# PlatonB/ld-tools

Measured on AMD Instinct MI355X. Metric: SNP-pairs/sec (r2+D'), higher is better.
Workload: dtype fp4 (E2M1 0/1 operands, exact f32 accumulation)

## Files before the change

### include/ldx.h

```cpp
#ifndef LDX_H
#define LDX_H

#include <stddef.h>
#include <stdint.h>

#ifdef __cplusplus
extern "C" {
#endif

#define LDX_VERSION 102
#define LDX_SLAB_ROWS 128u
#define LDX_GROUP_ROWS 8u
#define LDX_CHUNK_HAPS 128u
#define LDX_UNIT_PAIRS (LDX_SLAB_ROWS * LDX_GROUP_ROWS)
#define LDX_CELL_OFFSET4(r8, c) ((r8) * LDX_SLAB_ROWS + (((c) & 31u) << 2) + ((c) >> 5))
#define LDX_CELL_OFFSET8(r8, c) ((r8) * LDX_SLAB_ROWS + (((c) >> 6) << 6) + (((c) & 31u) << 1) + (((c) >> 5) & 1u))
#define LDX_CELL_OFFSET(out_format, r8, c) ((out_format) == LDX_OUT_LD32 ? LDX_CELL_OFFSET8(r8, c) : LDX_CELL_OFFSET4(r8, c))
#define LDX_MAX_HAPS 10240u

#define LDX_OK 0
#define LDX_E_ARG (-1)
#define LDX_E_HIP (-2)
#define LDX_E_UNSUPPORTED (-3)
#define LDX_E_OVERFLOW (-4)
// ... 4 lines not shown

#define LDX_MEASURE_RSQ 0
#define LDX_MEASURE_DPRIME 1

typedef struct { float r_square; float d_prime; } ldx_ld32;
typedef struct { uint16_t r_square; uint16_t d_prime; } ldx_k16;
typedef struct { double r_square; double d_prime; } ldx_ld64;
#define LDX_LD32_BIG_BITS 0x7FC00B16u
#define LDX_K16_INT0 0x8000u
#define LDX_K16_BIG 0x7FFFu
#define LDX_OUT_LD32 0
#define LDX_OUT_K16 1
typedef struct { uint16_t value; } ldx_k16one;
#define LDX_OUT_K16_RSQ 2
#define LDX_OUT_K16_DPRIME 3
typedef struct { float r; } ldx_r32;
#define LDX_OUT_R32 4

typedef struct {
    uint32_t query;
    uint32_t oppos;
    float r_square;
    float d_prime;
} ldx_hit;

int ldx_version(void);
const char *ldx_last_error(void);
int ldx_device_count(void);
int ldx_device_arch(int device, char *buf, size_t buflen);

uint32_t ldx_n_slabs(uint32_t n_snps);
uint32_t ldx_n_chunks(uint32_t n_hap);
size_t ldx_plane_bytes(uint32_t n_snps, uint32_t n_hap);
uint32_t ldx_padded_snps(uint32_t n_snps);
uint64_t ldx_triangle_units(uint32_t n_snps);
uint64_t ldx_triangle_unit_of(uint32_t n_snps, uint32_t row, uint32_t col);
uint64_t ldx_triangle_tile_base(uint32_t n_snps, uint32_t tile);
uint64_t ldx_triangle_cell_index(uint32_t n_snps, uint32_t row, uint32_t col, int out_format);

int ldx_pack_codes_dev(const int8_t *codes, uint32_t n_snps, uint32_t n_hap, size_t ld_codes,
                       void *alt, void *ref, uint32_t *acnt, uint32_t *rcnt, void *stream);
int ldx_tile_plane_dev(const uint32_t *rowmajor, uint32_t n_snps, uint32_t n_hap, size_t ld_words,
                       void *tiled, uint32_t *cnt, void *stream);
int ldx_snp_stats_dev(const uint32_t *acnt, const uint32_t *rcnt, uint32_t n_snps, uint32_t n_hap,
                      double *fa, double *fr, double *q, void *stream);

int ldx_alt_freq4_dev(const uint32_t *acnt, uint32_t n_snps, uint32_t n_hap, double *freq4, void *stream);

int ldx_panel_select_dev(const void *alt_src, const void *ref_src, uint32_t n_snps_src, uint32_t n_hap_src,
                         const uint32_t *snp_idx, uint32_t n_snps_dst, const uint32_t *hap_idx, uint32_t n_hap_dst,
                         void *alt_dst, void *ref_dst, uint32_t *acnt_dst, uint32_t *rcnt_dst, void *stream);

int ldx_bed_unpack_dev(const uint8_t *bed, size_t row_bytes, uint32_t n_ind_src, uint32_t n_rows,
                       const uint32_t *ind_idx, uint32_t n_ind_dst, int alt_is_a2, uint32_t row0, uint32_t n_snps_panel,
                       void *alt, void *ref, uint32_t *acnt, uint32_t *rcnt, void *stream);
int ldx_bed_pack_dev(const void *alt, const void *ref, uint32_t n_snps, uint32_t n_hap, uint32_t row0, uint32_t n_rows,
                     uint8_t *bed, size_t row_bytes, int alt_is_a2, void *stream);

int ldx_pair_counts_dev(const void *alt_i, uint32_t n_i, const void *alt_j, uint32_t n_j,
                        uint32_t n_hap, uint32_t *n11, size_t ld, void *stream);

int ldx_ld_from_counts_dev(uint32_t n, size_t m, const uint32_t *n11, const uint32_t *a1,
                           const uint32_t *r1, const uint32_t *a2, const uint32_t *r2,
                           ldx_ld64 *raw, ldx_ld32 *rounded, uint8_t *flags, void *stream);
int ldx_ld_from_counts_ex_dev(uint32_t n, size_t m, const uint32_t *n11, const uint32_t *a1,
                              const uint32_t *r1, const uint32_t *a2, const uint32_t *r2,
                              ldx_ld64 *raw, double *k, ldx_ld32 *cells32, ldx_k16 *cells16, uint8_t *flags,
                              void *stream);

int ldx_ld_pairs_dev(const void *alt, const uint32_t *acnt, const uint32_t *rcnt, uint32_t n_snps, uint32_t n_hap,
                     const uint32_t *rows, const uint32_t *cols, size_t m, double *k, ldx_ld64 *raw,
                     uint8_t *flags, uint32_t *n11, void *stream);

int ldx_triangle_dev(const void *alt, const double *fa, const double *fr, const double *q,
                     uint32_t n_snps, uint32_t n_hap, uint64_t unit_begin, uint64_t unit_end,
                     ldx_ld32 *out, ldx_ld64 *out_raw, uint32_t *out_n11, void *stream);
#define LDX_PATH_AUTO 0
#define LDX_PATH_POPCOUNT 1
#define LDX_PATH_MFMA 2
#define LDX_PATH_FP4 3
int ldx_set_triangle_path(int path);
int ldx_get_triangle_path(void);
size_t ldx_triangle_workspace_bytes(void);
int ldx_triangle_workspace_init_dev(void *workspace, size_t workspace_bytes, void *stream);
int ldx_triangle_ex_dev(const void *alt, const double *fa, const double *fr, const double *q,
                        uint32_t n_snps, uint32_t n_hap, uint64_t unit_begin, uint64_t unit_end,
                        int path, int out_format, void *out, ldx_ld64 *out_raw, uint32_t *out_n11,
                        void *workspace, size_t workspace_bytes, void *stream);

int ldx_triangle_dense_dev(const ldx_ld32 *strips, uint32_t n_snps, int measure, int has_thres,
                           double thres, uint32_t row_begin, uint32_t row_end, float *dense,
                           size_t ld, void *stream);
int ldx_triangle_dense_ex_dev(const void *strips, int strips_format, uint32_t n_snps, int measure, int has_thres,
                              double thres, uint32_t row_begin, uint32_t row_end, float *dense,
                              size_t ld, void *stream);
int ldx_triangle_r_block_dev(const ldx_r32 *strips, uint32_t n_snps, const uint32_t *acnt, const uint32_t *rcnt,
                             uint32_t n_hap, uint32_t row_begin, uint32_t row_end, uint32_t col_begin, uint32_t col_end,
                             float *out, size_t ld_out, void *stream);

int ldx_area_dev(const void *alt, const double *fa, const double *fr, const double *q,
                 uint32_t n_snps, uint32_t n_hap, const int64_t *positions,
                 const uint32_t *queries, uint32_t n_query, int64_t flank, int measure,
                 double thres, ldx_hit *hits, uint64_t hit_cap, uint64_t *n_hits, void *workspace,
                 size_t workspace_bytes, void *stream);
size_t ldx_area_workspace_bytes(uint32_t n_snps, uint32_t n_hap, uint32_t n_query);
int ldx_area_scan_dev(const void *alt, const double *fa, const double *fr, const double *q,
                      uint32_t n_snps, uint32_t n_hap, const int64_t *positions,
                      const uint32_t *queries, uint32_t n_query, int64_t flank, int measure,
                      double thres, ldx_hit *hits, uint64_t hit_cap, uint64_t *n_hits, uint32_t *query_counts,
                      void *workspace, size_t workspace_bytes, void *stream);
int ldx_area_finish_dev(ldx_hit *raw, const uint64_t *n_reserved, uint64_t hit_cap, uint32_t n_snps,
                        ldx_hit *sorted, uint32_t *offsets, uint64_t *summary, void *workspace,
                        size_t workspace_bytes, void *stream);
size_t ldx_area_finish_workspace_bytes(uint32_t n_snps);
int ldx_area_finish_ex_dev(ldx_hit *raw, const uint64_t *n_reserved, uint64_t hit_cap, uint32_t n_snps,
                           ldx_hit *sorted, uint32_t *offsets, uint64_t *summary, void *workspace,
                           size_t workspace_bytes, int counts_ready, void *stream);
uint32_t *ldx_area_finish_counts(void *finish_workspace);
int ldx_area_results_dev(const ldx_hit *sorted, uint64_t n_hits, int64_t *query, int64_t *oppos, float *values,
                         const uint32_t *offsets_src, uint32_t *offsets_dst, uint32_t n_offsets,
                         const uint32_t *word_src, uint32_t *word_dst, void *stream);
size_t ldx_area_band_passes_offset(uint32_t n_snps);
int ldx_set_area_path(int path);
int ldx_get_area_path(void);

size_t ldx_ld_score_workspace_bytes(uint32_t n_snps, uint32_t n_hap);
int ldx_ld_score_dev(const void *alt, const uint32_t *acnt, const uint32_t *rcnt, const double *fa, const double *fr,
                     uint32_t n_snps, uint32_t n_hap, const int64_t *positions, int64_t window,
                     const uint8_t *annot, uint32_t n_annot, int path,
                     uint64_t *sums, void *workspace, size_t workspace_bytes, void *stream);

#define LDX_DECAY_MAX_BINS 1024u
size_t ldx_ld_decay_workspace_bytes(uint32_t n_snps, uint32_t n_hap);
int ldx_ld_decay_dev(const void *alt, const uint32_t *acnt, const uint32_t *rcnt, const double *fa, const double *fr,
                     uint32_t n_snps, uint32_t n_hap, const int64_t *positions, int64_t window, int64_t bin_width,
                     const uint8_t *keep, int path,
                     uint64_t *sums, uint64_t *counts, uint32_t n_bins,
                     void *workspace, size_t workspace_bytes, void *stream);

size_t ldx_ld_fgt_workspace_bytes(uint32_t n_snps, uint32_t n_hap);
int ldx_ld_fgt_dev(const void *alt, const uint32_t *acnt, uint32_t n_snps, uint32_t n_hap, const int64_t *positions,
                   int64_t window, uint32_t min_count, const uint8_t *keep, int path,
                   uint32_t *left, void *workspace, size_t workspace_bytes, void *stream);
int ldx_ld_blocks_dev(const uint32_t *left, const int64_t *positions, const uint8_t *keep, uint32_t n_snps, int64_t window,
                      uint32_t *block_of, uint32_t *n_out, void *stream);

size_t ldx_ld_cross_workspace_bytes(uint32_t n_snps, uint32_t n_hap);
int ldx_ld_cross_dev(const void *alt, const uint32_t *acnt, const uint32_t *rcnt, const double *fa, const double *fr,
                     uint32_t n_snps, uint32_t n_hap, const int64_t *positions, int64_t window, int path,
                     uint64_t *sides, uint64_t *cross, void *workspace, size_t workspace_bytes, void *stream);
int ldx_ld_cross_scan_dev(const uint64_t *sides, uint32_t n_snps, uint64_t *cross, void *stream);
size_t ldx_ld_split_workspace_bytes(uint32_t n);
int ldx_ld_split_dev(const uint64_t *cross, uint32_t n, uint32_t min_snps, uint32_t max_snps,
                     uint32_t *cuts, uint32_t *n_out, void *workspace, size_t workspace_bytes, void *stream);

size_t ldx_ld_matvec_workspace_bytes(uint32_t n_snps, uint32_t n_hap);
int ldx_ld_matvec_dev(const void *alt, const uint32_t *acnt, const uint32_t *rcnt, const double *fa, const double *fr,
                      uint32_t n_snps, uint32_t n_hap, const int64_t *positions, int64_t window,
                      const float *x, uint32_t n_rhs, int power, int path,
                      int64_t *sums, void *workspace, size_t workspace_bytes, void *stream);

size_t ldx_ld_neighbors_workspace_bytes(uint32_t n_snps, uint32_t n_hap);
int ldx_ld_neighbors_dev(const void *alt, const uint32_t *acnt, const uint32_t *rcnt, const double *fa, const double *fr,
                         uint32_t n_snps, uint32_t n_hap, const int64_t *positions, int64_t window, float r2_bound, int path,
                         ldx_hit *hits, uint64_t hit_cap, uint64_t *n_hits, uint32_t *row_counts,
                         void *workspace, size_t workspace_bytes, void *stream);
// ... 94 lines not shown
                               const void *alt_j, const void *ref_j, const uint32_t *acnt_j, const uint32_t *rcnt_j, uint32_t n_j,
                               uint32_t n_hap, float r2_bound, ldx_hit *hits, uint64_t hit_cap, uint64_t *n_hits, void *stream);
int ldx_ld_em_pw_counts_dev(const void *alt_i, const void *ref_i, const uint32_t *acnt_i, const uint32_t *rcnt_i, uint32_t n_i,
                            const void *alt_j, const void *ref_j, const uint32_t *acnt_j, const uint32_t *rcnt_j, uint32_t n_j,
                            uint32_t n_hap, uint32_t *counts, size_t ld, void *stream);
int ldx_ld_em_from_counts_pw_dev(size_t m, const uint32_t *N, const uint32_t *a1, const uint32_t *a2, const uint32_t *S,
                                 const uint32_t *H, float *r, float *dprime, double *x, void *stream);

size_t ldx_ld_em_band_workspace_bytes(uint32_t n_snps);
int ldx_em_snp_stats_dev(const void *alt, const void *ref, const uint32_t *acnt, const uint32_t *rcnt, uint32_t n_snps,
                         uint32_t n_hap, int pairwise, uint32_t *N, uint32_t *A, float *diag, uint8_t *live, void *stream);
int ldx_ld_em_band_dev(const void *alt, const void *ref, const uint32_t *acnt, const uint32_t *rcnt, uint32_t n_snps,
                       uint32_t n_hap, int pairwise, const int64_t *positions, int64_t window, const uint32_t *lo,
                       const uint64_t *offsets, float *values_r, float *values_dprime, uint64_t n_cells, void *workspace,
                       size_t workspace_bytes, void *stream);
int ldx_ld_em_neighbors_dev(const void *alt, const void *ref, const uint32_t *acnt, const uint32_t *rcnt, uint32_t n_snps,
                            uint32_t n_hap, int pairwise, const int64_t *positions, int64_t window, float r2_bound,
                            ldx_hit *hits, uint64_t hit_cap, uint64_t *n_hits, void *workspace, size_t workspace_bytes,
                            void *stream);

typedef struct ldx_gabriel_params {
    uint32_t cand_cut, strong_hi, recomb_hi;
    uint32_t cut[4];
    int64_t max_span[4];
    uint32_t min_informative[4];
    uint32_t frac_num, frac_den;
} ldx_gabriel_params;
void ldx_gabriel_default_params(ldx_gabriel_params *params);
int ldx_ld_ci_from_counts_dev(size_t m, const uint32_t *N, const uint32_t *a1, const uint32_t *a2, const uint32_t *S,
                              const uint32_t *H, uint8_t *lo, uint8_t *hi, void *stream);
int ldx_ld_em_ci_band_dev(const void *alt, const void *ref, const uint32_t *acnt, const uint32_t *rcnt, uint32_t n_snps,
                          uint32_t n_hap, int pairwise, const int64_t *positions, int64_t window, const uint8_t *keep,
                          const uint32_t *lo, const uint64_t *offsets, uint8_t *ci_lo, uint8_t *ci_hi, uint64_t n_cells,
                          void *workspace, size_t workspace_bytes, void *stream);
size_t ldx_gabriel_candidates_workspace_bytes(uint32_t n_snps, uint64_t n_cells);
size_t ldx_gabriel_pick_workspace_bytes(uint32_t n_snps);
int ldx_gabriel_candidates_dev(const uint8_t *ci_lo, const uint8_t *ci_hi, const uint32_t *lo, const uint64_t *offsets,
                               uint64_t n_cells, const int64_t *positions, const uint8_t *keep, uint32_t n_snps, int64_t window,
                               const ldx_gabriel_params *params, int64_t *cand_span, uint32_t *cand_first, uint32_t *cand_last,
                               void *workspace, size_t workspace_bytes, void *stream);
int ldx_gabriel_pick_dev(const int64_t *sorted_span, const int64_t *order, const uint32_t *cand_first, const uint32_t *cand_last,
                         uint64_t n_cells, const uint8_t *keep, uint32_t n_snps, uint32_t *block_of, uint32_t *n_out,
                         void *workspace, size_t workspace_bytes, void *stream);

#define LDX_KING_MIN_SLICE_SNPS 65536u
#define LDX_KING_MAX_SLICE_SNPS 8388608u
#define LDX_KING_MAX_STORE_SNPS 134217728u
size_t ldx_sample_planes_bytes(uint32_t n_ind, uint32_t n_snps);
size_t ldx_sample_tables_bytes(uint32_t n_ind);
int ldx_sample_planes_dev(const void *alt, const void *ref, uint32_t n_snps, uint32_t n_hap, const uint8_t *keep,
                          uint32_t snp_begin, uint32_t snp_count, void *store, uint32_t *tables, void *stream);
int ldx_sample_counts_dev(const void *store, const uint32_t *tables, uint32_t n_ind, uint32_t n_snps, uint32_t *counts,
                          size_t ld, int accumulate, uint64_t n_prior, uint32_t n_slices, void *stream);
int ldx_king_from_counts_dev(size_t m, const uint32_t *N, const uint32_t *HH, const uint32_t *IBS0, const uint32_t *HETa,
                             const uint32_t *HETb, float *kin, float *ibs, void *stream);
int ldx_sample_cells_dev(const uint32_t *counts, uint32_t n_ind, size_t ld, float *kin, float *ibs, size_t ld_out, void *stream);

#define LDX_GENO_MAX_COLS 64u
#define LDX_GENO_MAX_SLICE_SNPS 4194304u
int ldx_geno_matmul_dev(const void *store, const uint32_t *tables, uint32_t n_ind, uint32_t n_snps, const int32_t *w,
                        const int32_t *wc, size_t ld_w, uint32_t k, int64_t *y, size_t ld_y, int accumulate, uint32_t n_slices,
                        void *stream);
int ldx_geno_rmatmul_dev(const void *alt, const void *ref, uint32_t n_snps, uint32_t n_hap, const uint8_t *keep,
                         const int32_t *u, size_t ld_u, uint32_t k, int64_t *z, int64_t *zc, size_t ld_z, void *stream);

int ldx_synth_codes_dev(int8_t *codes, uint32_t n_snps, uint32_t n_hap, size_t ld_codes,
                        uint64_t seed, const uint64_t *thresholds, uint64_t rho_thr,
                        uint32_t block_len, uint64_t miss_thr, uint32_t snp_offset, void *stream);
int ldx_synth_codes_ex_dev(int8_t *codes, uint32_t n_snps, uint32_t n_hap, size_t ld_codes,
                           uint64_t seed, const uint64_t *thresholds, uint64_t rho_thr,
                           uint32_t block_len, uint64_t miss_thr, uint32_t snp_offset,
                           uint64_t mono_thr, uint64_t miss_rows_thr, void *stream);

int ldx_calc_ld_host(const int8_t *g1, uint32_t h1, const int8_t *g2, uint32_t h2,
                     uint32_t counts[6], ldx_ld64 *raw, ldx_ld64 *rounded, double freq4[2],
                     uint8_t *flags);

int ldx_probe_andpop_dev(uint32_t *sink, uint32_t blocks, uint32_t threads, uint32_t iters, void *stream);

int ldx_probe_mfma_dev(uint32_t *sink, uint32_t blocks, uint32_t threads, uint32_t iters, int variant,
                       void *stream);

int ldx_debug_force_short_passes(int n_short);
int ldx_debug_counters(uint64_t out[8], int reset);

#ifdef __cplusplus
}
#endif
#endif
```

### ld_tools_amd/_lib.py

```python
from __future__ import annotations

import ctypes as C
import os
from pathlib import Path

from . import build as _build

LIB_PATH = Path(os.environ.get("LDX_LIB") or Path(__file__).resolve().parent / "libldx.so")

SLAB_ROWS = 128
GROUP_ROWS = 8
UNIT_PAIRS = SLAB_ROWS * GROUP_ROWS


def cell_offset(r8, c, fmt="k16"):
    if fmt in ("k16", "k16r", "k16d", "r32"):
        return r8 * SLAB_ROWS + ((c & 31) << 2) + (c >> 5)
    if fmt != "ld32":
        raise ValueError(f"unknown cell format {fmt!r}")
    return r8 * SLAB_ROWS + ((c >> 6) << 6) + ((c & 31) << 1) + ((c >> 5) & 1)


MAX_HAPS = 10240
DECAY_MAX_BINS = 1024
KING_MIN_SLICE_SNPS = 65536
KING_MAX_SLICE_SNPS = 1 << 23
KING_MAX_STORE_SNPS = 1 << 27
GENO_MAX_COLS = 64
GENO_MAX_SLICE_SNPS = 1 << 22
FLAG_DPRIME_INT0 = 1
FLAG_RSQ_INT0 = 2
MEASURES = {"r_square": 0, "d_prime": 1}
FORMATS = {"ld32": 0, "k16": 1, "k16r": 2, "k16d": 3,
           "r32": 4}
ONE_MEASURE = {"k16r": "r_square", "k16d": "d_prime"}
ONE_MEASURE_FMT = {v: k for k, v in ONE_MEASURE.items()}
LD32_BIG_BITS = 0x7FC00B16
K16_INT0 = 0x8000
K16_BIG = 0x7FFF
INVALID_ROW = 0xFFFFFFFF

E_NAMES = {-1: "LDX_E_ARG", -2: "LDX_E_HIP", -3: "LDX_E_UNSUPPORTED", -4: "LDX_E_OVERFLOW"}


class LdxError(RuntimeError):
    pass


def _load() -> C.CDLL:
    if not LIB_PATH.exists():
        try:
            _build.build(verbose=False)
        except Exception as exc:
            if not LIB_PATH.exists():
                raise ImportError(
                    f"ld_tools_amd: {LIB_PATH} is missing and could not be built ({exc}); "
                    "run `python ld_tools_amd/build.py` on a machine with hipcc. "
                    "There is no CPU fallback.") from exc
    _share_hip_runtime()
    return C.CDLL(str(LIB_PATH))


def _share_hip_runtime() -> None:
    try:
        import torch
    except ImportError:
        return
    cand = Path(torch.__file__).resolve().parent / "lib" / "libamdhip64.so"
    if cand.exists():
        C.CDLL(str(cand), mode=C.RTLD_GLOBAL)


lib = _load()

_vp, _u32, _u64, _i64, _sz, _int, _dbl = (C.c_void_p, C.c_uint32, C.c_uint64, C.c_int64, C.c_size_t,
                                          C.c_int, C.c_double)

SIGNATURES = {
    "ldx_version": (_int, []),
    "ldx_last_error": (C.c_char_p, []),
    "ldx_device_count": (_int, []),
    "ldx_device_arch": (_int, [_int, C.c_char_p, _sz]),
    "ldx_n_slabs": (_u32, [_u32]),
    "ldx_n_chunks": (_u32, [_u32]),
    "ldx_plane_bytes": (_sz, [_u32, _u32]),
    "ldx_padded_snps": (_u32, [_u32]),
    "ldx_triangle_units": (_u64, [_u32]),
    "ldx_triangle_unit_of": (_u64, [_u32, _u32, _u32]),
    "ldx_triangle_tile_base": (_u64, [_u32, _u32]),
    "ldx_triangle_cell_index": (_u64, [_u32, _u32, _u32, C.c_int]),
    "ldx_pack_codes_dev": (_int, [_vp, _u32, _u32, _sz, _vp, _vp, _vp, _vp, _vp]),
    "ldx_tile_plane_dev": (_int, [_vp, _u32, _u32, _sz, _vp, _vp, _vp]),
    "ldx_snp_stats_dev": (_int, [_vp, _vp, _u32, _u32, _vp, _vp, _vp, _vp]),
    "ldx_alt_freq4_dev": (_int, [_vp, _u32, _u32, _vp, _vp]),
    "ldx_panel_select_dev": (_int, [_vp, _vp, _u32, _u32, _vp, _u32, _vp, _u32, _vp, _vp, _vp, _vp, _vp]),
    "ldx_bed_unpack_dev": (_int, [_vp, _sz, _u32, _u32, _vp, _u32, _int, _u32, _u32, _vp, _vp, _vp, _vp, _vp]),
    "ldx_bed_pack_dev": (_int, [_vp, _vp, _u32, _u32, _u32, _u32, _vp, _sz, _int, _vp]),
    "ldx_pair_counts_dev": (_int, [_vp, _u32, _vp, _u32, _u32, _vp, _sz, _vp]),
    "ldx_ld_from_counts_dev": (_int, [_u32, _sz, _vp, _vp, _vp, _vp, _vp, _vp, _vp, _vp, _vp]),
    "ldx_triangle_dev": (_int, [_vp, _vp, _vp, _vp, _u32, _u32, _u64, _u64, _vp, _vp, _vp, _vp]),
    "ldx_triangle_ex_dev": (_int, [_vp, _vp, _vp, _vp, _u32, _u32, _u64, _u64, _int, _int, _vp, _vp, _vp, _vp, _sz, _vp]),
    "ldx_triangle_workspace_bytes": (_sz, []),
    "ldx_triangle_workspace_init_dev": (_int, [_vp, _sz, _vp]),
    "ldx_triangle_dense_ex_dev": (_int, [_vp, _int, _u32, _int, _int, _dbl, _u32, _u32, _vp, _sz, _vp]),
    "ldx_triangle_r_block_dev": (_int, [_vp, _u32, _vp, _vp, _u32, _u32, _u32, _u32, _u32, _vp, _sz, _vp]),
    "ldx_ld_from_counts_ex_dev": (_int, [_u32, _sz, _vp, _vp, _vp, _vp, _vp, _vp, _vp, _vp, _vp, _vp, _vp]),
    "ldx_ld_pairs_dev": (_int, [_vp, _vp, _vp, _u32, _u32, _vp, _vp, _sz, _vp, _vp, _vp, _vp, _vp]),
    "ldx_debug_force_short_passes": (_int, [_int]),
    "ldx_debug_counters": (_int, [_vp, _int]),
    "ldx_set_triangle_path": (_int, [_int]),
    "ldx_get_triangle_path": (_int, []),
    "ldx_triangle_dense_dev": (_int, [_vp, _u32, _int, _int, _dbl, _u32, _u32, _vp, _sz, _vp]),
    "ldx_area_dev": (_int, [_vp, _vp, _vp, _vp, _u32, _u32, _vp, _vp, _u32, _i64, _int, _dbl, _vp, _u64,
                            _vp, _vp, _sz, _vp]),
    "ldx_area_scan_dev": (_int, [_vp, _vp, _vp, _vp, _u32, _u32, _vp, _vp, _u32, _i64, _int, _dbl, _vp, _u64,
                                 _vp, _vp, _vp, _sz, _vp]),
    "ldx_area_workspace_bytes": (_sz, [_u32, _u32, _u32]),
    "ldx_area_finish_dev": (_int, [_vp, _vp, _u64, _u32, _vp, _vp, _vp, _vp, _sz, _vp]),
    "ldx_area_finish_ex_dev": (_int, [_vp, _vp, _u64, _u32, _vp, _vp, _vp, _vp, _sz, _int, _vp]),
    "ldx_area_finish_counts": (_vp, [_vp]),
    "ldx_area_results_dev": (_int, [_vp, _u64, _vp, _vp, _vp, _vp, _vp, _u32, _vp, _vp, _vp]),
    "ldx_area_finish_workspace_bytes": (_sz, [_u32]),
    "ldx_area_band_passes_offset": (_sz, [_u32]),
    "ldx_ld_score_workspace_bytes": (_sz, [_u32, _u32]),
    "ldx_ld_score_dev": (_int, [_vp, _vp, _vp, _vp, _vp, _u32, _u32, _vp, _i64, _vp, _u32, _int, _vp, _vp, _sz, _vp]),
    "ldx_ld_decay_workspace_bytes": (_sz, [_u32, _u32]),
    "ldx_ld_decay_dev": (_int, [_vp, _vp, _vp, _vp, _vp, _u32, _u32, _vp, _i64, _i64, _vp, _int, _vp, _vp, _u32, _vp, _sz, _vp]),
    "ldx_ld_fgt_workspace_bytes": (_sz, [_u32, _u32]),
    "ldx_ld_fgt_dev": (_int, [_vp, _vp, _u32, _u32, _vp, _i64, _u32, _vp, _int, _vp, _vp, _sz, _vp]),
    "ldx_ld_blocks_dev": (_int, [_vp, _vp, _vp, _u32, _i64, _vp, _vp, _vp]),
    "ldx_ld_cross_workspace_bytes": (_sz, [_u32, _u32]),
    "ldx_ld_cross_dev": (_int, [_vp, _vp, _vp, _vp, _vp, _u32, _u32, _vp, _i64, _int, _vp, _vp, _vp, _sz, _vp]),
    "ldx_ld_cross_scan_dev": (_int, [_vp, _u32, _vp, _vp]),
    "ldx_ld_split_workspace_bytes": (_sz, [_u32]),
    "ldx_ld_split_dev": (_int, [_vp, _u32, _u32, _u32, _vp, _vp, _vp, _sz, _vp]),
    "ldx_ld_matvec_workspace_bytes": (_sz, [_u32, _u32]),
    "ldx_ld_matvec_dev": (_int, [_vp, _vp, _vp, _vp, _vp, _u32, _u32, _vp, _i64, _vp, _u32, _int, _int, _vp, _vp, _sz, _vp]),
    "ldx_ld_neighbors_workspace_bytes": (_sz, [_u32, _u32]),
    "ldx_ld_neighbors_dev": (_int, [_vp, _vp, _vp, _vp, _vp, _u32, _u32, _vp, _i64, C.c_float, _int, _vp, _u64, _vp, _vp,
                                    _vp, _sz, _vp]),
    "ldx_dosage_stats_dev": (_int, [_vp, _vp, _u32, _u32, _vp, _vp, _vp]),
    "ldx_triangle_dosage_dev": (_int, [_vp, _vp, _u32, _u32, _u64, _u64, _int, _vp, _vp, _sz, _vp]),
    "ldx_triangle_r_block_dosage_dev": (_int, [_vp, _u32, _vp, _u32, _u32, _u32, _u32, _vp, _sz, _vp]),
    "ldx_ld_score_dosage_dev": (_int, [_vp, _vp, _u32, _u32, _vp, _i64, _vp, _u32, _int, _vp, _vp, _sz, _vp]),
    "ldx_ld_neighbors_dosage_dev": (_int, [_vp, _vp, _u32, _u32, _vp, _i64, C.c_float, _int, _vp, _u64, _vp, _vp, _vp, _sz,
                                           _vp]),
    "ldx_ld_band_layout_dev": (_int, [_vp, _u32, _i64, _vp, _vp, _vp]),
    "ldx_ld_band_workspace_bytes": (_sz, [_u32, _u32]),
    "ldx_ld_band_dev": (_int, [_vp, _vp, _vp, _vp, _vp, _u32, _u32, _vp, _i64, _int, _vp, _vp, _vp, _u64, _vp, _sz, _vp]),
    "ldx_ld_band_dosage_dev": (_int, [_vp, _vp, _u32, _u32, _vp, _i64, _int, _vp, _vp, _vp, _u64, _vp, _sz, _vp]),
    "ldx_band_score_dev": (_int, [_vp, _vp, _vp, _vp, _vp, _vp, _u32, _vp, _vp]),
    "ldx_band_matvec_dev": (_int, [_vp, _vp, _vp, _vp, _u32, _vp, _u32, _int, _vp, _vp]),
    "ldx_ld_rect_dev": (_int, [_vp, _vp, _vp, _u32, _vp, _vp, _vp, _u32, _u32, _vp, _sz, _vp]),
    "ldx_ld_rect_dosage_dev": (_int, [_vp, _vp, _u32, _vp, _vp, _u32, _u32, _vp, _sz, _vp]),
    "ldx_ld_rect_hits_dev": (_int, [_vp, _vp, _vp, _u32, _vp, _vp, _vp, _u32, _u32, C.c_float, _vp, _u64, _vp, _vp]),
    "ldx_ld_rect_hits_dosage_dev": (_int, [_vp, _vp, _u32, _vp, _vp, _u32, _u32, C.c_float, _vp, _u64, _vp, _vp]),
    "ldx_ld_rect_pw_dev": (_int, [_vp, _vp, _vp, _vp, _u32, _vp, _vp, _vp, _vp, _u32, _u32, _int, _vp, _sz, _vp]),
    "ldx_ld_rect_pw_hits_dev": (_int, [_vp, _vp, _vp, _vp, _u32, _vp, _vp, _vp, _vp, _u32, _u32, _int, C.c_float, _vp, _u64,
                                       _vp, _vp]),
    "ldx_ld_pw_band_workspace_bytes": (_sz, [_u32]),
    "ldx_pw_snp_stats_dev": (_int, [_vp, _vp, _vp, _vp, _u32, _u32, _int, _vp, _vp, _vp]),
    "ldx_ld_pw_band_dev": (_int, [_vp, _vp, _vp, _vp, _vp, _u32, _u32, _int, _vp, _i64, _vp, _vp, _vp, _u64, _vp, _sz, _vp]),
    "ldx_ld_pw_score_dev": (_int, [_vp, _vp, _vp, _vp, _vp, _u32, _u32, _int, _vp, _i64, _vp, _u32, _vp, _vp, _vp, _sz, _vp]),
    "ldx_ld_pw_neighbors_dev": (_int, [_vp, _vp, _vp, _vp, _vp, _u32, _u32, _int, _vp, _i64, C.c_float, _vp, _u64, _vp, _vp, _sz,
                                       _vp]),
    "ldx_ld_rect_pw_counts_dev": (_int, [_vp, _vp, _vp, _vp, _u32, _vp, _vp, _vp, _vp, _u32, _u32, _int, _vp, _sz, _vp]),
    "ldx_ld_em_rect_dev": (_int, [_vp, _vp, _u32, _vp, _vp, _u32, _u32, _vp, _vp, _sz, _vp]),
    "ldx_ld_em_rect_hits_dev": (_int, [_vp, _vp, _u32, _vp, _vp, _u32, _u32, C.c_float, _vp, _u64, _vp, _vp]),
    "ldx_ld_em_counts_dev": (_int, [_vp, _u32, _vp, _u32, _u32, _vp, _vp, _sz, _vp]),
    "ldx_ld_em_from_counts_dev": (_int, [_u32, _sz, _vp, _vp, _vp, _vp, _vp, _vp, _vp, _vp]),
    "ldx_ld_em_rect_pw_dev": (_int, [_vp, _vp, _vp, _vp, _u32, _vp, _vp, _vp, _vp, _u32, _u32, _vp, _vp, _sz, _vp]),
    "ldx_ld_em_rect_pw_hits_dev": (_int, [_vp, _vp, _vp, _vp, _u32, _vp, _vp, _vp, _vp, _u32, _u32, C.c_float, _vp, _u64, _vp,
                                          _vp]),
    "ldx_ld_em_pw_counts_dev": (_int, [_vp, _vp, _vp, _vp, _u32, _vp, _vp, _vp, _vp, _u32, _u32, _vp, _sz, _vp]),
    "ldx_ld_em_from_counts_pw_dev": (_int, [_sz, _vp, _vp, _vp, _vp, _vp, _vp, _vp, _vp, _vp]),
    "ldx_ld_em_band_workspace_bytes": (_sz, [_u32]),
    "ldx_em_snp_stats_dev": (_int, [_vp, _vp, _vp, _vp, _u32, _u32, _int, _vp, _vp, _vp, _vp, _vp]),
    "ldx_ld_em_band_dev": (_int, [_vp, _vp, _vp, _vp, _u32, _u32, _int, _vp, _i64, _vp, _vp, _vp, _vp, _u64, _vp, _sz, _vp]),
    "ldx_ld_em_neighbors_dev": (_int, [_vp, _vp, _vp, _vp, _u32, _u32, _int, _vp, _i64, C.c_float, _vp, _u64, _vp, _vp, _sz, _vp]),
    "ldx_gabriel_default_params": (None, [_vp]),
    "ldx_ld_ci_from_counts_dev": (_int, [_sz, _vp, _vp, _vp, _vp, _vp, _vp, _vp, _vp]),
    "ldx_ld_em_ci_band_dev": (_int, [_vp, _vp, _vp, _vp, _u32, _u32, _int, _vp, _i64, _vp, _vp, _vp, _vp, _vp, _u64, _vp, _sz, _vp]),
    "ldx_gabriel_candidates_workspace_bytes": (_sz, [_u32, _u64]),
    "ldx_gabriel_pick_workspace_bytes": (_sz, [_u32]),
    "ldx_gabriel_candidates_dev": (_int, [_vp, _vp, _vp, _vp, _u64, _vp, _vp, _u32, _i64, _vp, _vp, _vp, _vp, _vp, _sz, _vp]),
# ... 41 lines not shown
```

### ld_tools_amd/build.py

```python
from __future__ import annotations

import os
import shutil
import subprocess
import sys
from pathlib import Path

PKG = Path(__file__).resolve().parent
CSRC = PKG / "csrc"
LIB = PKG / "libldx.so"
SOURCES = ["ldx_api.hip", "ldx_pack.hip", "ldx_pairs.hip", "ldx_mfma.hip", "ldx_area.hip", "ldx_synth.hip",
           "ldx_select.hip", "ldx_band.hip", "ldx_rect.hip", "ldx_em.hip", "ldx_pwc.hip", "ldx_pwband.hip",
           "ldx_emband.hip", "ldx_bed.hip", "ldx_gabriel.hip", "ldx_king.hip", "ldx_geno.hip"]
HEADERS = [CSRC / "ldx_common.h", CSRC / "ldx_fp4.h", CSRC / "ldx_tile.h", CSRC / "ldx_pwc_tile.h", CSRC / "ldx_em_tile.h",
           CSRC / "ldx_em_pw_tile.h", CSRC / "ldx_band_plan.h", CSRC / "ldx_sample_store.h",
           PKG.parent / "include" / "ldx.h"]

FLAGS = ["-O3", "-std=c++17", "-fPIC", "-shared", "--offload-arch=gfx950", "-ffp-contract=off",
         "-fno-fast-math", "-fno-slp-vectorize", "-Wall", "-Wno-unused-function"]


def hipcc() -> str:
    exe = shutil.which("hipcc") or "/opt/rocm/bin/hipcc"
    if not os.path.exists(exe):
        raise RuntimeError("hipcc not found: cannot build libldx.so")
    return exe


def source_digest() -> str:
    import hashlib

    h = hashlib.sha256()
    for f in sorted([CSRC / s for s in SOURCES] + HEADERS):
        h.update(f.name.encode())
        h.update(f.read_bytes())
    return h.hexdigest()[:16]


def stale() -> bool:
    if not LIB.exists():
        return True
    t = LIB.stat().st_mtime
    deps = [CSRC / s for s in SOURCES] + HEADERS + [Path(__file__)]
    return any(d.stat().st_mtime > t for d in deps)


def build(force: bool = False, save_temps: bool = False, verbose: bool = True, out: Path = LIB,
          defines=()) -> Path:
    if not force and not stale() and out == LIB:
        return LIB
    tmp_lib = out.with_name(f"{out.name}.tmp.{os.getpid()}")
    cwd = PKG / "build"
    cwd.mkdir(exist_ok=True)
    tag = f"{out.stem}.{os.getpid()}"
    objs = [cwd / f"{Path(s).stem}.{tag}.o" for s in SOURCES]
    compile_flags = [f for f in FLAGS if f != "-shared"]
    extra = ["-save-temps=cwd", "-Rpass-analysis=kernel-resource-usage"] if save_temps else []
    cmds = [[hipcc(), *compile_flags, *defines, *extra, "-c", str(CSRC / s), "-o", str(o)] for s, o in zip(SOURCES, objs)]
    link = [hipcc(), "-shared", "-fPIC", "--offload-arch=gfx950", *[str(o) for o in objs], "-o", str(tmp_lib)]
    if verbose:
        for c in cmds + [link]:
            print("[ldx build]", " ".join(c), file=sys.stderr)
    try:
        from concurrent.futures import ThreadPoolExecutor

        def run(c):
            return subprocess.run(c, cwd=str(cwd), capture_output=not verbose and not save_temps, text=True)

        with ThreadPoolExecutor(max_workers=min(len(cmds), os.cpu_count() or 1)) as pool:
            results = list(pool.map(run, cmds))
        for c, r in zip(cmds, results):
            if r.returncode != 0:
                raise RuntimeError(f"hipcc failed ({r.returncode}): {' '.join(c)}\n{r.stderr or ''}")
        subprocess.run(link, check=True, cwd=str(cwd))
        os.replace(tmp_lib, out)
    finally:
        for f in [tmp_lib, *objs]:
            if f.exists():
                f.unlink()
    return out


if __name__ == "__main__":
    out = LIB
    if "--out" in sys.argv:
        out = PKG / sys.argv[sys.argv.index("--out") + 1]
    print(build(force="--force" in sys.argv, save_temps="--save-temps" in sys.argv, out=out,
                defines=[a for a in sys.argv[1:] if a.startswith("-D")]))
```

### ld_tools_amd/csrc/ldx_common.h

```cpp
#pragma once

#include <hip/hip_runtime.h>
#include <stdint.h>
#include <stdio.h>

#include <type_traits>

#include "../../include/ldx.h"

namespace ldx {

constexpr uint32_t kSlab = LDX_SLAB_ROWS;
constexpr uint32_t kGroup = LDX_GROUP_ROWS;
constexpr uint32_t kGroupsPerSlab = kSlab / kGroup;

void set_error(const char *fmt, ...);

__device__ __forceinline__ void block_sync()
{
    asm volatile("s_waitcnt lgkmcnt(0)" ::: "memory");
    __syncthreads();
}

template <typename T>
__device__ __forceinline__ void store_agent(T *p, T v)
{
    __hip_atomic_store(p, v, __ATOMIC_RELAXED, __HIP_MEMORY_SCOPE_AGENT);
}

double thres_to_k(double thres);

constexpr int kNoMatrixPath = -1000;

size_t triangle_mfma_workspace_bytes();
int triangle_mfma(const void *alt, const double *fa, const double *fr, const double *q, uint32_t n_snps, uint32_t n_hap,
                  uint64_t unit_begin, uint64_t unit_end, int out_format, void *out, ldx_ld64 *out_raw, uint32_t *out_n11,
                  bool fp4, void *workspace, hipStream_t s);

size_t area_mfma_workspace_bytes(uint32_t n_snps);
int area_mfma(const void *alt, const double *fa, const double *fr, const double *q, uint32_t n_snps, uint32_t n_hap,
              const int64_t *positions, const uint32_t *queries, uint32_t n_query, int64_t flank, int measure, double thres,
              ldx_hit *hits, uint64_t hit_cap, uint64_t *n_hits, uint32_t *query_counts, void *workspace, bool fp4,
              hipStream_t s);

#define LDX_HIP(call)                                                                       \
    do {                                                                                    \
        hipError_t e_ = (call);                                                             \
        if (e_ != hipSuccess) {                                                             \
            ::ldx::set_error("%s failed: %s (%s:%d)", #call, hipGetErrorString(e_), __FILE__, \
                             __LINE__);                                                     \
            return LDX_E_HIP;                                                               \
        }                                                                                   \
    } while (0)

#define LDX_REQUIRE(cond, msg)                                     \
    do {                                                           \
        if (!(cond)) {                                             \
            ::ldx::set_error("%s: %s", __func__, msg);             \
            return LDX_E_ARG;                                      \
        }                                                          \
    } while (0)

#define LDX_ARG_REQUIRE(cond, ...)           \
    do {                                     \
        if (!(cond)) {                       \
            ::ldx::set_error(__VA_ARGS__);   \
            return LDX_E_ARG;                \
        }                                    \
    } while (0)
#define LDX_ARG_PTR(who, ptr) LDX_ARG_REQUIRE((ptr) != nullptr, "%s: %s is a null pointer", who, #ptr)

int plane_check(const char *who, const char *arg, uint32_t n_snps, uint32_t n_hap);
int rect_args_ok(const char *who, uint32_t n_i, uint32_t n_j, uint32_t n_hap, const char *odd_reason, uint32_t tile_rows);
int hit_args_ok(const char *who, float r2_bound, const ldx_hit *hits, uint64_t hit_cap, const uint64_t *n_hits);

__host__ __device__ inline uint32_t n_slabs(uint32_t n_snps) { return (n_snps + kSlab - 1) / kSlab; }
__host__ __device__ inline uint32_t n_chunks(uint32_t n_hap) { return (n_hap + 255u) / 256u * 2u; }

__host__ __device__ inline uint64_t tile_base(uint64_t t, uint64_t G) { return t * G - 8u * t * (t - 1u); }

constexpr uint32_t kHitBatch = 256;
constexpr uint32_t kHitInvalid = 0xFFFFFFFFu;
struct HitAppender {
    ldx_hit *hits;
    uint64_t hit_cap;
    unsigned long long *n_hits;
    uint32_t lane;
    uint32_t *counts = nullptr;
    uint64_t slot = 0, slot_end = 0;

    __device__ __forceinline__ void close() const
    {
        for (uint64_t sl = slot + lane; sl < slot_end; sl += 64u)
            if (sl < hit_cap) hits[sl].query = kHitInvalid;
    }
    __device__ __forceinline__ void append(bool keep, uint32_t i, uint32_t j, float a, float b)
    {
        const unsigned long long mask = __ballot(keep);
        if (!mask) return;
        const uint32_t cnt = __builtin_popcountll(mask);
        if (slot + cnt > slot_end) {
            close();
            unsigned long long base = 0;
            if (lane == 0) base = atomicAdd(n_hits, (unsigned long long)kHitBatch);
            base = ((unsigned long long)__builtin_amdgcn_readfirstlane((uint32_t)(base >> 32)) << 32) |
                   __builtin_amdgcn_readfirstlane((uint32_t)base);
            slot = base;
            slot_end = base + kHitBatch;
        }
        if (keep) {
            const uint64_t sl = slot + __builtin_popcountll(mask & ((1ull << lane) - 1ull));
            if (sl < hit_cap) {
                hits[sl] = ldx_hit{i, j, a, b};
                if (counts) atomicAdd(&counts[i], 1u);
            }
        }
        slot += cnt;
    }
    __device__ __forceinline__ void append_both(bool keep, uint32_t i, uint32_t j, float a, float b)
    {
// ... 483 lines not shown
```

### ld_tools_amd/csrc/ldx_mfma.hip

```cpp
#include <stdlib.h>
#include <string.h>

#include <atomic>
#include <type_traits>

#include "ldx_common.h"
#include "ldx_fp4.h"
#include "ldx_tile.h"

namespace ldx {

typedef int v16i __attribute__((ext_vector_type(16)));
typedef unsigned v4u __attribute__((ext_vector_type(4)));
typedef unsigned v2u __attribute__((ext_vector_type(2)));
typedef float v4f __attribute__((ext_vector_type(4)));

__device__ __forceinline__ void gload16_s(v4u &dst, uint32_t voff, const void *sbase)
{
    const void *t;
    asm volatile("s_mov_b64 %1, %3\n\tglobal_load_dwordx4 %0, %2, %1" : "=v"(dst), "=&s"(t) : "v"(voff), "s"(sbase));
}
__device__ __forceinline__ void gload16x2_s(v4u &dst0, v4u &dst1, uint32_t voff, const void *sbase)
{
    const void *t;
    asm volatile("s_mov_b64 %2, %4\n\tglobal_load_dwordx4 %0, %3, %2\n\tglobal_load_dwordx4 %1, %3, %2 offset:512"
                 : "=&v"(dst0), "=&v"(dst1), "=&s"(t) : "v"(voff), "s"(sbase));
}
__device__ __forceinline__ void gload8_s(v2u &dst, uint32_t voff, const void *sbase)
{
    const void *t;
    asm volatile("s_mov_b64 %1, %3\n\tglobal_load_dwordx2 %0, %2, %1" : "=v"(dst), "=&s"(t) : "v"(voff), "s"(sbase));
}

#ifndef LDX_STEP_UNROLL
#define LDX_STEP_UNROLL 1
#endif
#ifndef LDX_VALU_PER_MFMA
#define LDX_VALU_PER_MFMA 5
#endif
constexpr int kMfmaWaves = 4;
constexpr int kMfmaThreads = kMfmaWaves * 64;
constexpr uint32_t kRows64 = 64;
constexpr uint32_t kBRow = 144;
constexpr uint32_t kBBuf = kSlab * kBRow;
constexpr uint32_t kStat = 6;
[[maybe_unused]] constexpr uint32_t kStampPasses = 40, kStampStride = 6 + 4 * kStampPasses + 20;


__device__ __forceinline__ v4i expand16(uint32_t bits)
{
    v4i r;
    r.x = (int)(((bits & 0xFu) * 0x00208208u) & 0x01020408u);
    r.y = (int)((((bits >> 4) & 0xFu) * 0x00208208u) & 0x01020408u);
    r.z = (int)((((bits >> 8) & 0xFu) * 0x00208208u) & 0x01020408u);
    r.w = (int)((((bits >> 12) & 0xFu) * 0x00208208u) & 0x01020408u);
    return r;
}

__device__ __forceinline__ v4i expand16_a(uint32_t word, uint32_t sel0, uint32_t sel1)
{
    const uint32_t p0 = __builtin_amdgcn_perm(word, word, sel0), p1 = __builtin_amdgcn_perm(word, word, sel1);
    v4i r;
    r.x = (int)(p0 & 0x08040201u);
    r.y = (int)((p0 >> 4) & 0x08040201u);
    r.z = (int)(p1 & 0x08040201u);
    r.w = (int)((p1 >> 4) & 0x08040201u);
    return r;
}

template <bool kDosage>
__device__ __forceinline__ v4i expand_b_fp4(uint32_t w)
{
    if constexpr (kDosage) return expand32_b4_dosage(w);
    else return expand32_b4(w);
}

#ifdef LDX_AB_NOAEXP
#define EXPAND_A(x) v4i{(int)(x), 1, 1, 1}
#else
#define EXPAND_A(x) expand16_a(x, sel0, sel1)
#endif
#ifdef LDX_AB_NOBEXP
#define EXPAND_B(x) v4i{(int)(x), 1, 1, 1}
#else
#define EXPAND_B(x) expand16(x)
#endif
#ifdef LDX_AB_NOBWRITE
#define BWRITE(dst, x) asm volatile("" : : "v"(x))
#else
#define BWRITE(dst, x) dst = (kFp4 ? expand_b_fp4<kDosage>(x) : EXPAND_B(x))
#endif

#ifdef LDX_CHUNK_STAMPS
#define LDX_CSTAMP(k)                                                                  \
    if (c_ == (uint32_t)(LDX_CHUNK_STAMPS) && npass == 1) asm volatile("s_memtime %0" : "=s"(cst[k]));
#else
#define LDX_CSTAMP(k)
#endif

__device__ __forceinline__ void expand_b_share(uint2 bits, unsigned char *buf, uint32_t tid)
{
    v4i *dst = reinterpret_cast<v4i *>(buf + (tid >> 1) * kBRow + (tid & 1u) * 64u);
    dst[0] = expand16(bits.x);
    dst[1] = expand16(bits.x >> 16);
    dst[2] = expand16(bits.y);
    dst[3] = expand16(bits.y >> 16);
}

__host__ __device__ inline uint32_t mfma_pass_base(uint32_t t, uint32_t n_slabs)
{
    auto c = [](uint32_t k) { return ((k + 1u) / 2u) * ((k + 2u) / 2u); };
    return c(n_slabs) - c(n_slabs - t);
}

constexpr uint32_t kCuSlots = 2048;
constexpr uint32_t kSchedWords = 3u + kCuSlots;
constexpr size_t kTriWorkspaceBytes = (kSchedWords * 4u + 255u) / 256u * 256u;
__device__ unsigned long long g_dbg[8];
#if defined(LDX_TUNING) && !defined(LDX_STAMPS_ONLY)
#define LDX_COUNT(slot, v) do { if (lane == 0) atomicAdd(&g_dbg[slot], (unsigned long long)(v)); } while (0)
#else
#define LDX_COUNT(slot, v)
#endif
static std::atomic<int> g_forced_short{-1};


enum class BandOp { None, Hits, Score, Cross, Nbr, Prod, Decay, Fgt, Store };

struct AreaArgs {
    const int64_t *pos;
    const uint8_t *is_query;
    const uint32_t *pass_base;
    const uint32_t *g_begin;
    const uint32_t *g_end;
    const uint32_t *order;
    ldx_hit *hits;
    uint32_t *counts;
    unsigned long long *n_hits;
    uint64_t hit_cap;
    double flank, k_thres;
    int measure;
    F32Const f32;
};
static_assert(sizeof(AreaArgs) == 112, "AreaArgs must not grow: see the comment inside it");
constexpr uint32_t kAreaDecoded = 1u << 30;
constexpr uint32_t kAreaQueue = 256;
#ifdef LDX_MM1
constexpr uint32_t kQueueCap = 32;
#else
constexpr uint32_t kQueueCap = 128;
#endif
constexpr size_t mfma_lds_bytes(uint32_t stat_rows, bool f32_tier, bool band_f32 = false)
{
    return 2u * kBBuf + (kSlab + kMfmaWaves * stat_rows) * kStat * sizeof(double) + 32u +
           (f32_tier ? (kSlab + kMfmaWaves * kRows64) * 16u + kMfmaWaves * kQueueCap * 36u + kMfmaWaves * 64u * 4u : 0u) +
           (band_f32 ? (kSlab + kMfmaWaves * kRows64) * 16u + kMfmaWaves * kAreaQueue * 8u : 0u);
}

#ifdef LDX_MM1
constexpr int kWgPerCu = 3;
constexpr uint32_t kStatRows = 32;
#else
constexpr int kWgPerCu = 2;
constexpr uint32_t kStatRows = kRows64;
#endif
template <typename Cell>
__device__ __forceinline__ void store_cell(Cell *p, Cell v)
{
    if constexpr (sizeof(Cell) == 2)
        __builtin_nontemporal_store(__builtin_bit_cast(uint16_t, v), reinterpret_cast<uint16_t *>(p));
    else if constexpr (sizeof(Cell) == 4)
        __builtin_nontemporal_store(__builtin_bit_cast(uint32_t, v), reinterpret_cast<uint32_t *>(p));
    else
        __builtin_nontemporal_store(__builtin_bit_cast(unsigned long long, v), reinterpret_cast<unsigned long long *>(p));
}

template <typename Cell>
__device__ __forceinline__ void store_words2_saddr(Cell *sbase, uint32_t voff_bytes, uint32_t w0, uint32_t w1)
{
    Cell *t;
    const v2u v = {w0, w1};
    asm volatile("s_mov_b64 %0, %3\n\tglobal_store_dwordx2 %1, %2, %0 nt" : "=&s"(t) : "v"(voff_bytes), "v"(v), "s"(sbase) : "memory");
}

template <int kOffset, typename Cell>
__device__ __forceinline__ void store_cell_saddr(Cell *sbase, uint32_t voff_bytes, Cell v)
{
    Cell *t;
    if constexpr (sizeof(Cell) == 4)
        asm volatile("s_mov_b64 %0, %3\n\tglobal_store_dword %1, %2, %0 offset:%4 nt" : "=&s"(t) : "v"(voff_bytes), "v"(__builtin_bit_cast(uint32_t, v)), "s"(sbase), "n"(kOffset) : "memory");
    else
        asm volatile("s_mov_b64 %0, %3\n\tglobal_store_dwordx2 %1, %2, %0 offset:%4 nt" : "=&s"(t) : "v"(voff_bytes), "v"(__builtin_bit_cast(unsigned long long, v)), "s"(sbase), "n"(kOffset) : "memory");
}

template <typename Cell>
__device__ __forceinline__ void store_cells4_saddr(Cell *sbase, uint32_t voff_bytes, Cell c0, Cell c1, Cell c2, Cell c3)
{
    Cell *t;
    if constexpr (sizeof(Cell) == 4) {
        const v4u v = {__builtin_bit_cast(uint32_t, c0), __builtin_bit_cast(uint32_t, c1), __builtin_bit_cast(uint32_t, c2),
// ... 22 lines not shown
    LDX_DPP_ADD(0x111, 0xF)
    LDX_DPP_ADD(0x112, 0xF)
    LDX_DPP_ADD(0x114, 0xF)
    LDX_DPP_ADD(0x118, 0xF)
    LDX_DPP_ADD(0x142, 0xA)
#undef LDX_DPP_ADD
    return ((uint64_t)hi << 32) | lo;
}

#define LDX_HIT_APPENDER                                                                                            \
    uint64_t slot = hit_slot, slot_end = hit_slot_end;                                                              \
    auto append = [&](bool keep, uint32_t qrow, uint32_t orow, float rec_a, float rec_b) {                          \
        const unsigned long long mask = __ballot(keep);                                                             \
        if (!mask) return;                                                                        \
        const uint32_t cnt = __builtin_popcountll(mask);                                                            \
        if (slot + cnt > slot_end) {                                                                                \
            for (uint64_t sl = slot + lane; sl < slot_end; sl += 64u)                                               \
                if (sl < aa.hit_cap) aa.hits[sl].query = kHitInvalid;                                               \
            unsigned long long base = 0;                                                                            \
            if (lane == 0) base = atomicAdd(aa.n_hits, (unsigned long long)kHitBatch);                              \
            base = ((unsigned long long)__builtin_amdgcn_readfirstlane((uint32_t)(base >> 32)) << 32) |             \
                   __builtin_amdgcn_readfirstlane((uint32_t)base);                                                  \
            slot = base;                                                                                            \
            slot_end = base + kHitBatch;                                                                            \
        }                                                                                                           \
        if (keep) {                                                                                                 \
            const uint64_t sl = slot + __builtin_popcountll(mask & ((1ull << lane) - 1ull));                        \
            if (sl < aa.hit_cap) {                                                                                  \
                aa.hits[sl] = ldx_hit{qrow, orow, rec_a, rec_b};                                                    \
                if (aa.counts) atomicAdd(&aa.counts[qrow], 1u);                                                     \
            }                                                                                                       \
        }                                                                                                           \
        slot += cnt;                                                                                                \
    };
#define LDX_BAND_LANE                                                                                               \
    uint32_t ln = lane;                                                                                             \
    asm volatile("" : "+v"(ln));                                                                                    \
    [[maybe_unused]] const uint32_t l32e = ln & 31u, halfe = ln >> 5;
#define LDX_BAND_COLS(l32x, per_col)                                                                                \
    [[maybe_unused]] double ca[4], cs[4], cpos[4];                                                                  \
    _Pragma("unroll") for (int tt = 0; tt < 4; ++tt) {                                                              \
        const d2s c0 = *reinterpret_cast<const d2s *>(cstat + (32u * tt + (l32x)) * kStat);                         \
        [[maybe_unused]] const d2s c1 = *reinterpret_cast<const d2s *>(cstat + (32u * tt + (l32x)) * kStat + 2u);   \
        ca[tt] = c0.x;                                                                                              \
        cs[tt] = c0.y;                                                                                              \
        cpos[tt] = c1.x;                                                                                            \
        per_col;                                                                                                    \
    }                                                                                                               \
    const uint32_t j0 = t * kSlab + (l32x);
#define LDX_BAND_SWEEP_BEGIN(halfx)                                                                                 \
    _Pragma("unroll 1") for (int e = 0; e < 16; ++e) {                                                              \
        _Pragma("unroll") for (int m = 0; m < 2; ++m) {                                                             \
            accel_t c4[4];                                                                                          \
            _Pragma("unroll") for (int tt = 0; tt < 4; ++tt) {                                                      \
                c4[tt] = acc[m][tt][e];                                                                             \
                asm volatile("" : "+v"(c4[tt]));                                                                    \
            }                                                                                                       \
            [[maybe_unused]] const uint32_t rlo = 32u * m + (uint32_t)(e & 3) + 8u * (uint32_t)(e >> 2);            \
            const uint32_t ri = rlo + 4u * (halfx);                                                                 \
            const d2s r0 = *reinterpret_cast<const d2s *>(rstat + ri * kStat);                                      \
            [[maybe_unused]] const d2s r1 = *reinterpret_cast<const d2s *>(rstat + ri * kStat + 2u);                \
            const uint32_t i = row0 + ri;
#define LDX_BAND_SWEEP_END                                                                                          \
        }                                                                                                           \
    }

template <bool kRaw, bool kN11, BandOp kOp = BandOp::None, bool kFp4 = false, typename Cell = ldx_ld32, int kSweep = 0,
          bool kDosage = false>
__global__ void __launch_bounds__(kMfmaThreads, kOp != BandOp::None ? 2 : kWgPerCu)
triangle_mfma_kernel(const uint4 *__restrict__ alt, const double *__restrict__ fa, const double *__restrict__ fr,
                     const double *__restrict__ q, uint32_t n_snps, uint32_t n_slabs, uint32_t nchunks, double n,
                     double rn, uint64_t u_begin, uint64_t u_end, Cell *__restrict__ out, ldx_ld64 *__restrict__ raw,
                     uint32_t *__restrict__ n11, uint32_t p_begin, uint32_t p_end_arg, uint32_t n_short, uint32_t *sched,
                     int ablate_arg, unsigned long long *stamps, AreaArgs aa)
{
    constexpr bool kArea = kOp != BandOp::None;
    constexpr bool kCross = kOp == BandOp::Cross;
    constexpr bool kScore = kOp == BandOp::Score || kCross;
    constexpr bool kNbr = kOp == BandOp::Nbr, kProd = kOp == BandOp::Prod, kDecay = kOp == BandOp::Decay;
    constexpr bool kFgt = kOp == BandOp::Fgt, kStore = kOp == BandOp::Store;
    static_assert((kSweep != 0) == (kScore || kProd), "kSweep: the words (Score, Cross) or right-hand sides (Prod) per accumulator sweep");
    static_assert(!kCross || kSweep == 1, "the one-sided sums are the score band's column 0, rows and columns apart");
    const uint32_t p_end = kArea ? aa.pass_base[n_slabs] : p_end_arg;
    const uint32_t n_norm = p_end - p_begin - n_short, n_tickets = n_norm + 2u * n_short;
#if defined(LDX_TUNING) && !defined(LDX_STAMPS_ONLY)
    int ablate = ablate_arg;
    if (ablate_arg & 64) ablate = (blockIdx.x < (gridDim.x + 1) / 2) ? 5 : 2;
    if ((ablate_arg & 128) && blockIdx.x >= (gridDim.x + 1) / 2) return;
#else
    constexpr int ablate = 0;
    (void)ablate_arg;
    (void)stamps;
#endif
    extern __shared__ uint4 lds[];
    unsigned char *bexp = reinterpret_cast<unsigned char *>(lds);
    double *cstat = reinterpret_cast<double *>(bexp + 2u * kBBuf);
    const uint32_t tid = threadIdx.x;
    const uint32_t lane = tid & 63u;
    const uint32_t l32 = lane & 31u;
    const uint32_t half = lane >> 5;
    const uint32_t sel0 = half ? 0x02020202u : 0x00000000u;
    const uint32_t sel1 = half ? 0x03030303u : 0x01010101u;
    const uint32_t wave = __builtin_amdgcn_readfirstlane(tid >> 6);
    double *rstat = cstat + kSlab * kStat + wave * ((kArea ? kRows64 : kStatRows) * kStat);
    const FastConst fk = fast_const(n, kFp4 ? 1.0 : 8.0);
#ifdef LDX_TUNING
    uint32_t npass = 0;
    unsigned long long *const my_stamps = stamps ? stamps + (size_t)(blockIdx.x * kMfmaWaves + wave) * kStampStride : nullptr;
    if (my_stamps && lane == 0) {
        my_stamps[0] = (unsigned long long)__builtin_amdgcn_s_getreg(63492) |
                       ((unsigned long long)__builtin_amdgcn_s_getreg(63508) << 32);
        my_stamps[1] = __builtin_amdgcn_s_memrealtime();
        my_stamps[2] = __builtin_amdgcn_s_memtime();
    }
#define LDX_STAMP(slot)                                                                                    \
    do {                                                                                                   \
        if (my_stamps && lane == 0 && npass < kStampPasses) my_stamps[6 + npass * 4 + (slot)] = __builtin_amdgcn_s_memtime(); \
    } while (0)
#else
#define LDX_STAMP(slot)
#endif

    const uint64_t G64 = (uint64_t)n_slabs * 2u;
    auto base64 = [&](uint64_t t) { return t * G64 - t * (t - 1u); };
    const uint64_t v_begin = u_begin / 8u, v_end = (u_end + 7u) / 8u;

    uint32_t *tickets = reinterpret_cast<uint32_t *>(cstat + kSlab * kStat + kMfmaWaves * ((kArea ? kRows64 : kStatRows) * kStat));
    uint32_t *cols_odd = tickets + 2;
    constexpr bool kR32 = std::is_same<Cell, ldx_r32>::value;
    constexpr bool kF32Tier = kFp4 && !kRaw && !kN11 && !kArea && !kR32;
    static_assert(!kDosage || (kFp4 && ((kR32 && !kArea) || kOp == BandOp::Score || kNbr || kStore)),
                  "dosage r: the FP4 r32 triangle, the LD-score band, the neighbour band and the band store");
    auto snp_ars = [&](uint32_t x) {
        if constexpr (kDosage) {
            const double *const g = fa + 2u * (size_t)x;
            return R32Snp{g[0], g[1]};
        } else {
            return r32_snp(fa[x], fr[x], n);
        }
    };
    constexpr bool kBandF32 = kFp4 && kOp == BandOp::Hits;
    float *ctab32 = reinterpret_cast<float *>(tickets + 8);
    float *rtab32 = ctab32 + kSlab * 4u + wave * (kRows64 * 4u);
    uint32_t *qid = reinterpret_cast<uint32_t *>(ctab32 + kSlab * 4u + kMfmaWaves * kRows64 * 4u) + wave * kQueueCap;
    float *qcnt = reinterpret_cast<float *>(reinterpret_cast<uint32_t *>(ctab32 + kSlab * 4u + kMfmaWaves * kRows64 * 4u) +
                                            kMfmaWaves * kQueueCap) + wave * (kQueueCap * 8u);
    uint32_t *ulist = reinterpret_cast<uint32_t *>(ctab32 + kSlab * 4u + kMfmaWaves * kRows64 * 4u) + kMfmaWaves * kQueueCap * 9u +
                      wave * 64u;
    uint32_t *aq_id = reinterpret_cast<uint32_t *>(ctab32 + kSlab * 4u + kMfmaWaves * kRows64 * 4u) + wave * kAreaQueue;
    uint32_t *aq_cnt = reinterpret_cast<uint32_t *>(ctab32 + kSlab * 4u + kMfmaWaves * kRows64 * 4u) + kMfmaWaves * kAreaQueue + wave * kAreaQueue;
    auto prod_rows = [&](uint32_t w) { return ctab32 + kMfmaWaves * kRows64 * 16u + w * (kRows64 * 8u); };
    uint64_t *const decay_sum = reinterpret_cast<uint64_t *>(ctab32);
    uint64_t *const store_off = reinterpret_cast<uint64_t *>(ctab32) + wave * (kRows64 * 3u / 2u);
    uint32_t *const store_lo = reinterpret_cast<uint32_t *>(store_off + kRows64);
    uint64_t *const decay_cnt = decay_sum + (kDecay ? (uint32_t)aa.measure : 0u);
    const F32Const fc32 = aa.f32;
    const uint32_t my_xcd = kArea ? (__builtin_amdgcn_s_getreg(63508) & 7u) : 0u;
    uint32_t static_next = blockIdx.x;
    auto draw = [&]() -> uint32_t {
        if constexpr (kArea) {
            for (uint32_t k = 0; k < 8u; ++k) {
                const uint32_t x = (my_xcd + k) & 7u;
                const uint32_t lo = aa.pass_base[(uint32_t)((uint64_t)n_slabs * x / 8u)], hi = aa.pass_base[(uint32_t)((uint64_t)n_slabs * (x + 1u) / 8u)];
                if (lo == hi) continue;
                const uint32_t got = atomicAdd(&sched[2u + 32u * x], 1u);
                if (got < hi - lo) return aa.order ? aa.order[lo + got] : lo + got;
            }
            return 0xFFFFFFFFu;
        } else {
            if (!sched) return static_next += gridDim.x;
            return gridDim.x + atomicAdd(&sched[0], 1u);
        }
    };
    uint32_t *ktok = nullptr;
    if (!kArea && sched && (ablate_arg & 4096)) {
        const uint32_t hw = __builtin_amdgcn_s_getreg(63492), xcc = __builtin_amdgcn_s_getreg(63508);
        ktok = sched + 2u + ((((xcc & 7u) * 8u + ((hw >> 13) & 7u)) * 2u + ((hw >> 12) & 1u)) * 16u + ((hw >> 8) & 15u));
    }
    uint32_t parity = 0;
    if constexpr (kDecay)
        for (uint32_t b = tid; b < 2u * (uint32_t)aa.measure; b += kMfmaThreads) decay_sum[b] = 0u;
    if (tid == 0) tickets[0] = kArea ? draw() : blockIdx.x;

    uint64_t hit_slot = 0, hit_slot_end = 0;
    uint32_t t_prev = 0xFFFFFFFFu;
    for (;;) {
        block_sync();
        const uint32_t ticket = tickets[parity];
        parity ^= 1u;
        if (kArea ? ticket == 0xFFFFFFFFu : ticket >= n_tickets) {
            if (tid == 0 && sched && atomicAdd(&sched[1], 1u) == gridDim.x - 1u) {
                store_agent(&sched[1], 0u);
                if (kArea)
                    for (uint32_t x = 0; x < 8u; ++x) store_agent(&sched[2u + 32u * x], 0u);
                asm volatile("s_waitcnt vmcnt(0)" ::: "memory");
                store_agent(&sched[0], 0u);
            }
            break;
        }
        const bool short_pass = !kArea && ticket >= n_norm;
        const uint32_t hsel = short_pass ? (ticket - n_norm) & 1u : 0u;
        const uint32_t seq = short_pass ? n_norm + ((ticket - n_norm) >> 1) : ticket;
        uint32_t p = p_begin + seq;
        auto pbase = [&](uint32_t tile) { return kArea ? aa.pass_base[tile] : mfma_pass_base(tile, n_slabs); };
        auto tile_of_pass = [&](uint32_t pp) {
            uint32_t lo = 0, hi = n_slabs;
            while (hi - lo > 1) {
                const uint32_t mid = (lo + hi) / 2;
                if (pbase(mid) <= pp) lo = mid; else hi = mid;
            }
            return lo;
        };
        uint32_t t;
        if (kArea && (ticket & kAreaDecoded)) {
            t = (ticket >> 12) & 0xFFFu;
            p = pbase(t) + (ticket & 0xFFFu);
        } else
#ifndef LDX_AB_FORWARD_TILES
        if constexpr (!kArea) {
            const uint32_t mirrored = p_end - 1u - seq;
            t = tile_of_pass(mirrored);
            const uint32_t lo_t = pbase(t) > p_begin ? pbase(t) : p_begin;
            const uint32_t hi_t = (t + 1u < n_slabs && pbase(t + 1u) < p_end) ? pbase(t + 1u) : p_end;
            p = lo_t + (hi_t - 1u - mirrored);
        } else
#endif
        {
            t = tile_of_pass(p);
        }
        const bool new_tile = t != t_prev;
        t_prev = t;
        const uint64_t tb = base64(t), te = base64(t + 1u);
        const uint64_t area_first = kArea ? tb + (aa.g_begin[t] - 2u * t) : 0u;
        const uint64_t pass = (kArea ? area_first : tb) + (uint64_t)(p - pbase(t)) * kMfmaWaves;
        const uint64_t seg_begin = kArea ? area_first : (v_begin > tb ? v_begin : tb);
        const uint64_t seg_end = kArea ? tb + (aa.g_end[t] > 2u * t ? aa.g_end[t] - 2u * t : 0u) : (v_end < te ? v_end : te);
        const uint32_t b_off = kFp4 ? ((tid >> 7) * kSlab + (tid & 127u)) * 16u : (tid >> 1) * kBRow + (tid & 1u) * 64u;
        const uint32_t nblocks = kFp4 ? nchunks / 2u : nchunks;

        auto pass_body = [&](auto mm_c) {
            constexpr int MM = decltype(mm_c)::value;
            const uint64_t vv = pass + wave;
            const bool active = vv >= seg_begin && vv < seg_end;
            const uint32_t g64 = (uint32_t)((vv < te ? vv : pass) - tb) + 2u * t;
            const uint32_t roff = MM == 1 ? 32u * hsel : 0u;
            const uint32_t row0 = g64 * kRows64 + roff;
            const bool pad_only = kF32Tier && row0 >= n_snps;
            const bool counting = active && !pad_only;
            const uint4 *ai = alt + ((size_t)(row0 / kSlab) * nchunks) * kSlab + (row0 % kSlab) + l32 + (kFp4 ? half * kSlab : 0u);
            constexpr uint32_t kAStride = kFp4 ? 2u * kSlab : kSlab;

            typedef std::conditional_t<kFp4, v16f, v16i> acc_t;
            typedef std::conditional_t<kFp4, float, int> accel_t;
            auto count_of = [](accel_t x) { if constexpr (kFp4) return (uint32_t)x; else return (uint32_t)x >> 3; };
            auto count_f64 = [](accel_t x) { if constexpr (kFp4) return (double)x; else return (double)((uint32_t)x >> 3); };
            acc_t acc[MM][4];
#pragma unroll
            for (int m = 0; m < MM; ++m)
#pragma unroll
                for (int tt = 0; tt < 4; ++tt)
#pragma unroll
                    for (int e = 0; e < 16; ++e) acc[m][tt][e] = 0;

            auto read_bf = [&](v4i (&bf)[4], const unsigned char *buf, int w) {
#pragma unroll
                for (int tt = 0; tt < 4; ++tt)
#ifdef LDX_AB_NOBREAD
                    bf[tt] = v4i{(int)(uintptr_t)buf + w + tt, 1, 1, 1};
#else
                    bf[tt] = kFp4 ? *reinterpret_cast<const v4i *>(buf + (((uint32_t)w * 2u + half) * kSlab + 32u * tt + l32) * 16u)
                                  : *reinterpret_cast<const v4i *>(buf + (32u * tt + l32) * kBRow + w * 32u + half * 16u);
#endif
            };
            auto mma8 = [&](const v4i (&af)[MM], const v4i (&bf)[4]) {
#pragma unroll
                for (int m = 0; m < MM; ++m)
#pragma unroll
                    for (int tt = 0; tt < 4; ++tt)
#ifdef LDX_AB_NOMFMA
                        asm volatile("" : "+v"(acc[m][tt]) : "v"(af[m]), "v"(bf[tt]));
#else
                    {
                        if constexpr (kFp4) {
                            const v8i a8v = {af[m].x, af[m].y, af[m].z, af[m].w, 0, 0, 0, 0};
                            const v8i b8v = {bf[tt].x, bf[tt].y, bf[tt].z, bf[tt].w, 0, 0, 0, 0};
                            acc[m][tt] = __builtin_amdgcn_mfma_scale_f32_32x32x64_f8f6f4(a8v, b8v, acc[m][tt], 4, 4, 0, 0, 0, 0);
                        } else {
                            acc[m][tt] = __builtin_amdgcn_mfma_i32_32x32x32_i8(af[m], bf[tt], acc[m][tt], 0, 0, 0);
                        }
                    }
#endif
            };
            auto interleave = [&]() {
                __builtin_amdgcn_sched_group_barrier(0x100, 4, 0);
#pragma unroll
                for (int k = 0; k < 4 * MM; ++k) {
                    __builtin_amdgcn_sched_group_barrier(0x008, 1, 0);
                    __builtin_amdgcn_sched_group_barrier(0x002, LDX_VALU_PER_MFMA, 0);
                }
            };
            auto lds_barrier = [&]() {
                __builtin_amdgcn_sched_barrier(0);
#ifndef LDX_AB_NOBARRIER
                __builtin_amdgcn_s_waitcnt(0xC07F);
                __builtin_amdgcn_s_barrier();
#endif
                __builtin_amdgcn_sched_barrier(0);
            };

            LDX_STAMP(0);
            v4u ar[3][MM];
            auto touch_ring = [&](int k) {
                if constexpr (MM == 2) asm volatile("" : "+v"(ar[k][0]), "+v"(ar[k][1]));
                else asm volatile("" : "+v"(ar[k][0]));
            };
            typedef std::conditional_t<kFp4, v4u, v2u> bring_t;
            bring_t br[3];
            auto clampc = [&](uint32_t c) { return c < nblocks ? c : nblocks - 1u; };
            constexpr uint32_t kBlockBytes = kAStride * 16u;
            const uint32_t b_voff = kFp4 ? (uint32_t)((((size_t)t * nchunks + (tid >> 7)) * kSlab + (tid & 127u)) * 16u)
                                         : (uint32_t)(((size_t)t * nchunks * kSlab) * 16u + tid * 8u);
            const uint32_t a_voff = (uint32_t)((size_t)(ai - alt) * 16u);
            auto block_base = [&](uint32_t blk) { return reinterpret_cast<const unsigned char *>(alt) + (size_t)blk * kBlockBytes; };
            auto load_b = [&](bring_t &dst, uint32_t blk) {
                if constexpr (kFp4) gload16_s(dst, b_voff, block_base(blk));
                else gload8_s(dst, b_voff, block_base(blk));
            };
            auto load_a = [&](v4u (&dst)[MM], uint32_t blk) {
                if constexpr (MM == 2) gload16x2_s(dst[0], dst[1], a_voff, block_base(blk));
                else gload16_s(dst[0], a_voff, block_base(blk));
            };
            auto bquarter = [&](unsigned char *buf, const bring_t &bits, int q) {
                if constexpr (kFp4) {
                    BWRITE(*reinterpret_cast<v4i *>(buf + b_off + (uint32_t)q * (2u * kSlab * 16u)), bits[q]);
                } else {
                    const uint32_t w = q < 2 ? bits.x : bits.y;
                    BWRITE(*reinterpret_cast<v4i *>(buf + b_off + (uint32_t)q * 16u), (q & 1) ? w >> 16 : w);
                }
            };
            auto expand_a = [&](uint32_t x) {
                if constexpr (kFp4) return expand32_a4(x);
                else return EXPAND_A(x);
            };
            {
                bring_t w0;
                load_b(w0, 0u);
                load_b(br[1], clampc(1));
#pragma unroll
                for (int k = 0; k < 2; ++k) load_a(ar[k], clampc(k));
                asm volatile("s_waitcnt vmcnt(0)");
                asm volatile("" : "+v"(w0), "+v"(br[1]));
                touch_ring(0);
                touch_ring(1);
#pragma unroll
                for (int q = 0; q < 4; ++q) bquarter(bexp, w0, q);
                bquarter(bexp + kBBuf, br[1], 0);
            }
            bool rows_ordinary = false;
            typedef double d2s __attribute__((ext_vector_type(2)));
            if constexpr (kFgt) {
                if (new_tile && tid < kSlab) {
                    const uint32_t j = t * kSlab + tid;
                    d2s *dst = reinterpret_cast<d2s *>(cstat + tid * kStat);
                    dst[0] = d2s{j < n_snps ? (double)aa.counts[j] : 0.0, 0.0};
                    dst[1] = j < n_snps ? d2s{(double)aa.pos[j], (double)aa.is_query[j]} : d2s{0.0, 0.0};
                }
                const uint32_t i = row0 + lane;
                d2s *dst = reinterpret_cast<d2s *>(rstat + lane * kStat);
                dst[0] = d2s{i < n_snps ? (double)aa.counts[i] : 0.0, 0.0};
                dst[1] = i < n_snps ? d2s{(double)aa.pos[i], (double)aa.is_query[i]} : d2s{0.0, 0.0};
            } else if constexpr (kStore) {
                if (new_tile && tid < kSlab) {
                    const R32Snp c = snp_ars(t * kSlab + tid);
                    *reinterpret_cast<d2s *>(cstat + tid * kStat) = d2s{c.a, c.rs};
                }
                const uint32_t i = row0 + lane;
                const R32Snp r = snp_ars(i);
                *reinterpret_cast<d2s *>(rstat + lane * kStat) = d2s{r.a, r.rs};
                store_lo[lane] = i < n_snps ? aa.counts[i] : 0xFFFFFFFFu;
                store_off[lane] = i < n_snps ? reinterpret_cast<const uint64_t *>(aa.is_query)[i] : 0u;
            } else if constexpr (kScore || kNbr || kProd || kDecay) {
                if (new_tile && tid < kSlab) {
                    const uint32_t j = t * kSlab + tid;
                    const R32Snp c = snp_ars(j);
                    d2s *dst = reinterpret_cast<d2s *>(cstat + tid * kStat);
                    dst[0] = d2s{c.a, c.rs};
                    dst[1] = j < n_snps ? d2s{(double)aa.pos[j], (double)(aa.is_query ? aa.is_query[j] : (uint8_t)0)} : d2s{0.0, 0.0};
                }
                const uint32_t i = row0 + lane;
                const R32Snp r = snp_ars(i);
                d2s *dst = reinterpret_cast<d2s *>(rstat + lane * kStat);
                dst[0] = d2s{r.a, r.rs};
                dst[1] = i < n_snps ? d2s{(double)aa.pos[i], (double)(aa.is_query ? aa.is_query[i] : (uint8_t)0)} : d2s{0.0, 0.0};
                if constexpr (kProd) {
                    const float *const x = reinterpret_cast<const float *>(aa.counts);
                    const uint32_t nr = (uint32_t)aa.measure & 15u;
                    float xr[8];
#pragma unroll
                    for (uint32_t k = 0; k < 8u; ++k) xr[k] = (i < n_snps && k < nr) ? x[(size_t)i * nr + k] : 0.0f;
                    v4f *xd = reinterpret_cast<v4f *>(prod_rows(wave) + lane * 8u);
                    xd[0] = v4f{xr[0], xr[1], xr[2], xr[3]};
                    xd[1] = v4f{xr[4], xr[5], xr[6], xr[7]};
                }
            } else if constexpr (kR32) {
                if (new_tile && tid < kSlab) {
                    const uint32_t j = t * kSlab + tid;
                    const R32Snp c = snp_ars(j);
                    *reinterpret_cast<d2s *>(cstat + tid * kStat) = d2s{c.a, c.rs};
                }
                const uint32_t i = row0 + (MM == 1 ? l32 : lane);
                const R32Snp r = snp_ars(i);
                if (lane < kStatRows) *reinterpret_cast<d2s *>(rstat + lane * kStat) = d2s{r.a, r.rs};
            } else if (!kRaw) {
                if (new_tile && tid < kSlab) {
                    const uint32_t j = t * kSlab + tid;
                    const FastCol c = fast_col(fa[j], fr[j], n);
                    const int ccls = snp_class(fa[j], fr[j], n);
                    const bool odd = ccls != kSnpOrdinary;
                    if (lane == 0) cols_odd[wave] = 0u;
                    if (__any(odd) && lane == 0) cols_odd[wave] = 1u;
                    typedef double d2 __attribute__((ext_vector_type(2)));
                    d2 *dst = reinterpret_cast<d2 *>(cstat + tid * kStat);
                    dst[0] = d2{c.a, c.ra};
                    dst[1] = d2{c.rr, c.rq};
                    if (kArea) dst[2] = j < n_snps ? d2{(double)aa.pos[j], (double)(aa.is_query ? aa.is_query[j] : (uint8_t)1)} : d2{0.0, 0.0};
                    if constexpr (kF32Tier) {
                        const F32Col c32 = f32_col(c.a, c.ra, c.rr, ccls, n);
                        *reinterpret_cast<v4f *>(ctab32 + tid * 4u) = v4f{c32.a, c32.ra, c32.rr, c32.s};
                    }
                    if constexpr (kBandF32) {
                        float ah, al;
                        f32_split_a((float)c.a, ah, al);
                        const double ar = 1.0 / c.rq;
                        const double kc = aa.k_thres - 2.5;
                        const double cthr = ar > 0.0 ? 0.1 * __builtin_sqrt((kc > 0.0 ? kc : 0.0) * ar) * (1.0 - 0x1p-20) : __builtin_inf();
                        *reinterpret_cast<v4f *>(ctab32 + tid * 4u) = v4f{ah, al, (float)cthr, 0.0f};
                    }
                }
                const uint32_t i = row0 + (MM == 1 ? l32 : lane);
                const FastRow r = fast_row(fa[i], fr[i], n);
                const int rcls = snp_class(fa[i], fr[i], n);
                rows_ordinary = __all(rcls == kSnpOrdinary);
                typedef double d2 __attribute__((ext_vector_type(2)));
                d2 *dst = reinterpret_cast<d2 *>(rstat + (lane < (kArea ? kRows64 : kStatRows) ? lane : 0u) * kStat);
                if (lane < (kArea ? kRows64 : kStatRows)) {
                    dst[0] = d2{r.a_s, r.ra};
                    dst[1] = d2{r.rr, r.rq_s};
                }
                if constexpr (kF32Tier) {
                    const F32Row r32 = f32_row(r.a_s * 1e-4, r.ra, r.rr, rcls, n);
                    *reinterpret_cast<v4f *>(rtab32 + lane * 4u) = v4f{r32.a, r32.ra_s, r32.rr_s, r32.s};
                }
                if constexpr (kBandF32) {
                    const double s1 = 10.0 * __builtin_sqrt(r.ra * r.rr);
                    *reinterpret_cast<v4f *>(rtab32 + lane * 4u) = v4f{(float)(r.a_s * 1e-4), s1 < __builtin_inf() ? (float)s1 : 0.0f, 0.0f, 0.0f};
                }
                if (kArea) dst[2] = i < n_snps ? d2{(double)aa.pos[i], (double)(aa.is_query ? aa.is_query[i] : (uint8_t)1)} : d2{0.0, 0.0};
            }
            if (ktok && tid == 0)
                while (atomicCAS(ktok, 0u, 1u) != 0u) __builtin_amdgcn_s_sleep(4);
            block_sync();
            LDX_STAMP(1);
            if (ablate & 32) __builtin_amdgcn_s_setprio(2);
#if defined(LDX_AB_BANDPRIO)
            if (kArea) { if (LDX_AB_BANDPRIO == 1 ? (blockIdx.x >= gridDim.x / 2u) : (blockIdx.x & 1u)) __builtin_amdgcn_s_setprio(1); else __builtin_amdgcn_s_setprio(0); }
#endif
            v4i af0[MM], bf0[4], af1[MM], bf1[4];
            read_bf(bf0, bexp, 0);
#pragma unroll
            for (int m = 0; m < MM; ++m) af0[m] = expand_a(ar[0][m].x);

            const uint32_t nch_run = (ablate & 2) ? 1u : nblocks;
#ifdef LDX_CHUNK_STAMPS
            unsigned long long cst[6] = {0, 0, 0, 0, 0, 0};
#endif
#define LDX_CHUNK(CUR, NXT, FAR, cc)                                                                               \
            {                                                                                                      \
                const uint32_t c_ = (cc);                                                                          \
                const unsigned char *rd = bexp + (c_ & 1u) * kBBuf;                                                \
                unsigned char *wr = bexp + ((c_ + 1u) & 1u) * kBBuf;                                               \
                const uint32_t c3 = clampc(c_ + 2u);                                                               \
                LDX_CSTAMP(0)                                                                                      \
                 \
                       \
                load_b(br[FAR], c3);                                                                               \
                load_a(ar[FAR], c3);                                                                               \
                asm volatile("s_waitcnt vmcnt(%0)" : : "n"(MM == 2 ? 5 : 3));    \
                asm volatile("" : "+v"(br[NXT]));                                                                  \
                      \
                read_bf(bf1, rd, 1);                                                                               \
                _Pragma("unroll") for (int m = 0; m < MM; ++m) af1[m] = expand_a(ar[CUR][m].y);               \
                bquarter(wr, br[NXT], 1);                                                                          \
                mma8(af0, bf0);                                                                                    \
                interleave();                                                                                      \
                __builtin_amdgcn_sched_barrier(0);                                                                 \
                LDX_CSTAMP(1)                                                                                      \
                                             \
                read_bf(bf0, rd, 2);                                                                               \
                _Pragma("unroll") for (int m = 0; m < MM; ++m) af0[m] = expand_a(ar[CUR][m].z);               \
                bquarter(wr, br[NXT], 2);                                                                          \
                mma8(af1, bf1);                                                                                    \
                interleave();                                                                                      \
                __builtin_amdgcn_sched_barrier(0);                                                                 \
                LDX_CSTAMP(2)                                                                                      \
                                             \
                read_bf(bf1, rd, 3);                                                                               \
                _Pragma("unroll") for (int m = 0; m < MM; ++m) af1[m] = expand_a(ar[CUR][m].w);               \
                bquarter(wr, br[NXT], 3);                                                                          \
                mma8(af0, bf0);                                                                                    \
                interleave();                                                                                      \
                __builtin_amdgcn_sched_barrier(0);                                                                 \
                LDX_CSTAMP(3)                                                                                      \
                lds_barrier();                        \
                LDX_CSTAMP(4)                                                                                      \
                   \
                 \
                           \
                asm volatile("s_waitcnt vmcnt(%0)" : : "n"(MM));                                                   \
                touch_ring(NXT);                                                                                   \
                asm volatile("" : "+v"(br[FAR]));                                                                  \
                read_bf(bf0, wr, 0);                                                                               \
                _Pragma("unroll") for (int m = 0; m < MM; ++m) af0[m] = expand_a(ar[NXT][m].x);               \
                bquarter(bexp + (c_ & 1u) * kBBuf, br[FAR], 0);                                                    \
                mma8(af1, bf1);                                                                                    \
                interleave();                                                                                      \
                __builtin_amdgcn_sched_barrier(0);                                                                 \
                LDX_CSTAMP(5)                                                                                      \
            }
#define LDX_CHUNK_IDLE(NXT, FAR, cc)                                                                               \
            {                                                                                                      \
                const uint32_t c_ = (cc);                                                                          \
                unsigned char *wr = bexp + ((c_ + 1u) & 1u) * kBBuf;                                               \
                load_b(br[FAR], clampc(c_ + 2u));                                                                  \
                asm volatile("s_waitcnt vmcnt(1)");                                 \
                asm volatile("" : "+v"(br[NXT]));                                                                  \
                bquarter(wr, br[NXT], 1);                                                                          \
                bquarter(wr, br[NXT], 2);                                                                          \
                bquarter(wr, br[NXT], 3);                                                                          \
                lds_barrier();                                                                                     \
                asm volatile("s_waitcnt vmcnt(0)");                                                                \
                asm volatile("" : "+v"(br[FAR]));                                                                  \
                bquarter(bexp + (c_ & 1u) * kBBuf, br[FAR], 0);                                                    \
            }
            if (__builtin_expect(!counting, 0)) {
                for (uint32_t c = 0; c < nch_run; c += 3) {
                    LDX_CHUNK_IDLE(1, 2, c)
                    if (c + 1 < nch_run) LDX_CHUNK_IDLE(2, 0, c + 1)
                    if (c + 2 < nch_run) LDX_CHUNK_IDLE(0, 1, c + 2)
                }
            } else {
#ifdef LDX_AB_PEEL
            if constexpr (!kArea) {
                LDX_CHUNK(0, 1, 2, 0u)
                for (uint32_t c = 1; c < nch_run; c += 3) {
                    LDX_CHUNK(1, 2, 0, c)
                    if (c + 1 < nch_run) LDX_CHUNK(2, 0, 1, c + 1)
                    if (c + 2 < nch_run) LDX_CHUNK(0, 1, 2, c + 2)
                }
            } else
#endif
            {
                for (uint32_t c = 0; c < nch_run; c += 3) {
                    LDX_CHUNK(0, 1, 2, c)
                    if (c + 1 < nch_run) LDX_CHUNK(1, 2, 0, c + 1)
                    if (c + 2 < nch_run) LDX_CHUNK(2, 0, 1, c + 2)
                }
            }
            }
#undef LDX_CHUNK
#undef LDX_CHUNK_IDLE
            asm volatile("s_waitcnt vmcnt(0)");
            touch_ring(0);
            touch_ring(1);
            touch_ring(2);
            asm volatile("" : "+v"(br[0]), "+v"(br[1]), "+v"(br[2]));

#ifdef LDX_CHUNK_STAMPS
            asm volatile("s_waitcnt lgkmcnt(0)");
            if (my_stamps && lane == 0 && npass == 1)
                for (int k = 0; k < 6; ++k) my_stamps[6 + 4 * (kStampPasses - 2) + k] = cst[k];
#endif
            LDX_STAMP(2);
            uint32_t next_ticket = 0;
            if (tid == 0) {
                if (ktok) atomicExch(ktok, 0u);
                next_ticket = draw();
            }
            if (ablate & 32) __builtin_amdgcn_s_setprio(0);
            else if (!(ablate & 16)) __builtin_amdgcn_s_setprio(3);
            if constexpr (kScore || kProd) {
                block_sync();
            } else if (!active) {
                if (tid == 0) tickets[parity] = next_ticket;
                return;
            }
            typedef double d2 __attribute__((ext_vector_type(2)));
            double fa2[4], fr2[4];
            double sfa = 0.0, sfr = 0.0, sq = 0.0;
#pragma unroll
            for (int tt = 0; tt < 4; ++tt) {
                if (kRaw) {
                    fa2[tt] = fa[t * kSlab + 32u * tt + l32];
                    fr2[tt] = fr[t * kSlab + 32u * tt + l32];
                }
            }
            if (kRaw) {
                const uint32_t il = row0 + (MM == 1 ? l32 : lane);
                sfa = fa[il];
                sfr = fr[il];
                sq = q[il];
            }
            auto epilogue = [&](auto clean_c) {
#pragma unroll 1
            for (int e = 0; e < 16; ++e) {
                constexpr bool kClean = decltype(clean_c)::value;
                uint32_t ri[MM], cnt[MM][4];
                uint64_t us[MM];
                bool in_range[MM], valid[MM][4], slow[MM][4];
                Cell res[MM][4];
                ldx_ld64 rw[MM][4];
                bool any_slow = false;
#pragma unroll
                for (int m = 0; m < MM; ++m) {
                    ri[m] = 32u * m + (e & 3) + 8u * (e >> 2) + 4u * half;
                    us[m] = vv * 8u + (ri[m] + roff) / kGroup;
                    in_range[m] = kClean || (us[m] >= u_begin && us[m] < u_end);
                }
                if (kRaw) {
#pragma unroll
                    for (int m = 0; m < MM; ++m) {
                        const uint32_t i = row0 + ri[m];
                        const double fa1 = __shfl(sfa, (int)ri[m]), fr1 = __shfl(sfr, (int)ri[m]), q1 = __shfl(sq, (int)ri[m]);
#pragma unroll
                        for (int tt = 0; tt < 4; ++tt) {
                            const uint32_t j = t * kSlab + 32u * tt + l32;
                            valid[m][tt] = (i > j) && (i < n_snps);
                            cnt[m][tt] = count_of(acc[m][tt][e]);
                            const LdRaw lr = ld_epilogue((double)cnt[m][tt] / n, fa1, fr1, q1, fa2[tt], fr2[tt]);
                            res[m][tt] = encode_cell<Cell>(round_pair(lr));
                            rw[m][tt] = valid[m][tt] ? ldx_ld64{lr.rsq, lr.dprime} : ldx_ld64{0.0, 0.0};
                        }
                    }
                } else {
                    FastRow fr2x[MM];
#pragma unroll
                    for (int m = 0; m < MM; ++m) {
                        const d2 *rs = reinterpret_cast<const d2 *>(rstat + ri[m] * kStat);
                        const d2 r01 = rs[0], r23 = rs[1];
                        fr2x[m] = FastRow{r01.x, r01.y, r23.x, r23.y};
                    }
                    constexpr int kPairs = MM == 2 ? 4 : 2;
                    auto chain_m = [](int, int k) { return MM == 2 ? k : 0; };
                    auto chain_tt = [](int pp, int k) { return MM == 2 ? pp : 2 * pp + k; };
                    auto load_col = [&](int tt) {
                        const d2 *cs = reinterpret_cast<const d2 *>(cstat + (32u * tt + l32) * kStat);
                        const d2 c01 = cs[0], c23 = cs[1];
                        return FastCol{c01.x, c01.y, c23.x, c23.y};
                    };
                    FastCol nxt[2];
                    nxt[0] = load_col(chain_tt(0, 0));
                    nxt[1] = MM == 2 ? nxt[0] : load_col(chain_tt(0, 1));
#pragma unroll
                    for (int pp = 0; pp < kPairs; ++pp) {
                        const FastCol fcx[2] = {nxt[0], nxt[1]};
                        if (pp + 1 < kPairs) {
                            nxt[0] = load_col(chain_tt(pp + 1, 0));
                            nxt[1] = MM == 2 ? nxt[0] : load_col(chain_tt(pp + 1, 1));
                        }
                        FastRow frk[2];
                        accel_t a8[2];
                        Cell r2[2];
                        bool s2[2];
#pragma unroll
                        for (int k = 0; k < 2; ++k) {
                            const int m = chain_m(pp, k), tt = chain_tt(pp, k);
                            frk[k] = fr2x[m];
                            const uint32_t i = row0 + ri[m], j = t * kSlab + 32u * tt + l32;
// ... 778 lines not shown
                        }
                        if (!(bm[0] | bm[1] | bm[2] | bm[3])) continue;
                        const unsigned long long lo01 = (bm[0] & 0xFFFFFFFFull) | (bm[1] << 32), lo23 = (bm[2] & 0xFFFFFFFFull) | (bm[3] << 32);
                        const unsigned long long hi01 = (bm[0] >> 32) | (bm[1] & 0xFFFFFFFF00000000ull), hi23 = (bm[2] >> 32) | (bm[3] & 0xFFFFFFFF00000000ull);
                        const uint32_t vlo = lo23 ? 128u - (uint32_t)__builtin_clzll(lo23) : (lo01 ? 64u - (uint32_t)__builtin_clzll(lo01) : 0u);
                        const uint32_t vhi = hi23 ? 128u - (uint32_t)__builtin_clzll(hi23) : (hi01 ? 64u - (uint32_t)__builtin_clzll(hi01) : 0u);
                        best = ln == rlo ? vlo : (ln == rlo + 4u ? vhi : best);
                LDX_BAND_SWEEP_END
                const uint32_t i = row0 + ln;
                if (best != 0u && i < n_snps) atomicMax(reinterpret_cast<uint32_t *>(aa.hits) + i, t * kSlab + best);
              }
            };
            auto store_epilogue = [&]() {
              if constexpr (kStore && MM == 2) {
                float *const values = reinterpret_cast<float *>(aa.hits);
                const uint64_t n_cells = aa.hit_cap;
                LDX_BAND_LANE
                LDX_BAND_COLS(l32e, )
                LDX_BAND_SWEEP_BEGIN(halfe)
                        const uint32_t lo_i = store_lo[ri];
                        const uint64_t off_i = store_off[ri];
#pragma unroll
                        for (int tt = 0; tt < 4; ++tt) {
                            const double cnt = count_f64(c4[tt]);
                            const float c = r32_cell(cnt, n, r0.x, r0.y, ca[tt], cs[tt]).r;
                            const uint32_t j = j0 + 32u * tt;
                            const uint64_t idx = off_i + (uint64_t)(j - lo_i);
                            if (j < i && j >= lo_i && idx < n_cells) __builtin_nontemporal_store(c, values + idx);
                        }
                LDX_BAND_SWEEP_END
              }
            };
            if constexpr (kScore || kProd) {
                const uint32_t st = kProd ? (uint32_t)aa.measure & 15u : 1u + (uint32_t)aa.measure;
                if constexpr (kProd) {
                    if (active) prod_epilogue(st, ((uint32_t)aa.measure & 16u) != 0u);
                } else {
                    if (active) score_epilogue(st);
                }
                block_sync();
                uint64_t *const sums = reinterpret_cast<uint64_t *>(aa.hits);
                for (uint32_t f = tid; f < kSlab * st; f += kMfmaThreads) {
                    uint64_t v = 0;
#pragma unroll
                    for (uint32_t w = 0; w < (uint32_t)kMfmaWaves; ++w)
                        if (pass + w >= seg_begin && pass + w < seg_end) v += score_cols[w * (kSlab * 9u) + f];
                    const uint32_t j = t * kSlab + f / st;
                    const size_t word = kCross ? (size_t)j * 2u + 1u : (size_t)j * st + f % st;
                    if (v != 0u && j < n_snps) atomicAdd(reinterpret_cast<unsigned long long *>(sums) + word, (unsigned long long)v);
                }
                finish_pass(std::false_type{});
                return;
            }
            if constexpr (kArea) {
                if constexpr (kNbr) nbr_epilogue();
                else if constexpr (kDecay) decay_epilogue();
                else if constexpr (kFgt) fgt_epilogue();
                else if constexpr (kStore) store_epilogue();
                else area_epilogue();
                finish_pass(std::true_type{});
                return;
            }
            const bool interior = row0 >= (t + 1u) * kSlab && row0 + 32u * MM <= n_snps && (t + 1u) * kSlab <= n_snps;
            const bool whole = vv * 8u >= u_begin && vv * 8u + 8u <= u_end;
            const bool inside = !kRaw && interior && whole;
            const bool all_ordinary = rows_ordinary && (cols_odd[0] | cols_odd[1]) == 0u;
            const bool clean = inside && all_ordinary;
            if constexpr (kR32) {
                epilogue_r32();
            } else if constexpr (kF32Tier) {
                if (whole && !(ablate & 512) && epilogue_f32(all_ordinary, !interior)) {
                } else if (clean && !(ablate & 512)) {
                    epilogue(std::true_type{});
                } else {
                    epilogue(std::false_type{});
                }
            } else {
                if (clean && !(ablate & 512)) epilogue(std::true_type{});
                else epilogue(std::false_type{});
            }
            finish_pass(std::true_type{});
        };
        if constexpr (kArea) {
            pass_body(std::integral_constant<int, 2>{});
        } else {
#ifdef LDX_MM1
            pass_body(std::integral_constant<int, 1>{});
#else
            if (short_pass) pass_body(std::integral_constant<int, 1>{});
            else pass_body(std::integral_constant<int, 2>{});
#endif
        }
    }
    if constexpr (kDecay) {
        unsigned long long *const gsum = reinterpret_cast<unsigned long long *>(aa.hits);
        unsigned long long *const gcnt = reinterpret_cast<unsigned long long *>(aa.counts);
        for (uint32_t b = tid; b < (uint32_t)aa.measure; b += kMfmaThreads) {
            const uint64_t c = decay_cnt[b];
            if (c != 0u) {
                atomicAdd(gsum + b, (unsigned long long)decay_sum[b]);
                atomicAdd(gcnt + b, (unsigned long long)c);
            }
        }
    }
    if (kArea && !kStore)
        for (uint64_t sl = hit_slot + lane; sl < hit_slot_end; sl += 64u)
            if (sl < aa.hit_cap) aa.hits[sl].query = kHitInvalid;
}

#undef LDX_HIT_APPENDER
#undef LDX_BAND_LANE
#undef LDX_BAND_COLS
#undef LDX_BAND_SWEEP_BEGIN
#undef LDX_BAND_SWEEP_END

template <bool kRaw, bool kN11, bool kFp4, typename Cell, bool kDosage = false>
static int launch_mfma(const void *alt, const double *fa, const double *fr, const double *q, uint32_t n_snps,
                       uint32_t n_hap, uint64_t unit_begin, uint64_t unit_end, Cell *out, ldx_ld64 *out_raw,
                       uint32_t *out_n11, uint32_t *sched, hipStream_t s)
{
    const uint32_t nch = n_chunks(n_hap);
    if (plane_check("ld_triangle on the matrix pipe", nullptr, n_snps, n_hap)) return kNoMatrixPath;
    const size_t lds = mfma_lds_bytes(kStatRows, kFp4 && !kRaw && !kN11 && !std::is_same<Cell, ldx_r32>::value);
    if (lds > 64u * 1024u) {
        static std::atomic<uint64_t> opted{0};
        int dev = 0;
        LDX_HIP(hipGetDevice(&dev));
        if (dev < 0 || dev >= 64 || !((opted.load(std::memory_order_relaxed) >> dev) & 1u)) {
            LDX_HIP(hipFuncSetAttribute((const void *)triangle_mfma_kernel<kRaw, kN11, BandOp::None, kFp4, Cell, 0, kDosage>,
                                        hipFuncAttributeMaxDynamicSharedMemorySize, (int)lds));
            if (dev >= 0 && dev < 64) opted.fetch_or(1ull << dev, std::memory_order_relaxed);
        }
    }
    const int cus = device_cus();
    const uint32_t ns = n_slabs(n_snps);
    const uint64_t G64 = (uint64_t)ns * 2u;
    auto base64 = [&](uint64_t t) { return t * G64 - t * (t - 1u); };
    auto tile_of = [&](uint64_t v) {
        uint32_t lo = 0, hi = ns;
        while (hi - lo > 1) {
            const uint32_t mid = (lo + hi) / 2;
            if (base64(mid) <= v) lo = mid; else hi = mid;
        }
        return lo;
    };
    const uint64_t v_begin = unit_begin / 8u, v_end = (unit_end + 7u) / 8u;
    const uint32_t t0 = tile_of(v_begin), t1 = tile_of(v_end - 1u);
    const uint32_t p_begin = mfma_pass_base(t0, ns) + (uint32_t)((v_begin - base64(t0)) / kMfmaWaves);
    const uint32_t p_end = mfma_pass_base(t1, ns) + (uint32_t)((v_end - base64(t1) + kMfmaWaves - 1u) / kMfmaWaves);
    const uint64_t slots = (uint64_t)cus * kWgPerCu;
    const uint32_t n_pass = p_end - p_begin;
    uint32_t n_short = 2ull * n_pass <= slots ? n_pass : (n_pass > slots ? (uint32_t)(slots / 4u) : 0u);
    const int forced = g_forced_short.load(std::memory_order_relaxed);
    if (forced >= 0) n_short = (uint32_t)forced < n_pass ? (uint32_t)forced : n_pass;
#ifdef LDX_MM1
    n_short = n_pass;
#endif
    uint64_t grid = slots;
    if (grid > (uint64_t)n_pass + n_short) grid = (uint64_t)n_pass + n_short;
    if (grid < 1) grid = 1;
    AreaArgs tri_args{};
    tri_args.f32 = f32_const((double)n_hap);
    int ablate = 0;
    unsigned long long *stamps = nullptr;
#ifdef LDX_TUNING
    ablate = getenv("LDX_ABLATE") ? atoi(getenv("LDX_ABLATE")) : 0;
    const char *stamp_file = getenv("LDX_STAMPS");
    const size_t stamp_words = (size_t)grid * kMfmaWaves * kStampStride;
    if (stamp_file) {
        LDX_HIP(hipMalloc(&stamps, stamp_words * 8));
        LDX_HIP(hipMemsetAsync(stamps, 0, stamp_words * 8, s));
    }
#endif
    const double n_obs = kDosage ? (double)(n_hap / 2u) : (double)n_hap;
    triangle_mfma_kernel<kRaw, kN11, BandOp::None, kFp4, Cell, 0, kDosage><<<(uint32_t)grid, kMfmaThreads, lds, s>>>(
        (const uint4 *)alt, fa, fr, q, n_snps, n_slabs(n_snps), nch, n_obs, 1.0 / n_obs, unit_begin,
        unit_end, out, out_raw, out_n11, p_begin, p_end, n_short, sched, ablate, stamps, tri_args);
    LDX_HIP(hipGetLastError());
#ifdef LDX_TUNING
    if (stamps) {
        unsigned long long *h = (unsigned long long *)malloc(stamp_words * 8);
        LDX_HIP(hipStreamSynchronize(s));
        LDX_HIP(hipMemcpy(h, stamps, stamp_words * 8, hipMemcpyDeviceToHost));
        if (FILE *f = fopen(stamp_file, "wb")) {
            const unsigned long long hdr[4] = {grid, (unsigned long long)kMfmaWaves, kStampStride, kStampPasses};
            fwrite(hdr, 8, 4, f);
            fwrite(h, 8, stamp_words, f);
            fclose(f);
        }
        free(h);
        LDX_HIP(hipFree(stamps));
    }
#endif
    return LDX_OK;
}

size_t triangle_mfma_workspace_bytes() { return kTriWorkspaceBytes; }

int triangle_mfma(const void *alt, const double *fa, const double *fr, const double *q, uint32_t n_snps, uint32_t n_hap,
                  uint64_t unit_begin, uint64_t unit_end, int out_format, void *out, ldx_ld64 *out_raw, uint32_t *out_n11,
                  bool fp4, void *workspace, hipStream_t s)
{
    uint32_t *const sched = (uint32_t *)workspace;
#define LDX_GO(R, N, CELL)                                                                                          \
    return fp4 ? launch_mfma<R, N, true, CELL>(alt, fa, fr, q, n_snps, n_hap, unit_begin, unit_end, (CELL *)out,    \
                                               out_raw, out_n11, sched, s)                                          \
               : launch_mfma<R, N, false, CELL>(alt, fa, fr, q, n_snps, n_hap, unit_begin, unit_end, (CELL *)out,   \
                                                out_raw, out_n11, sched, s)
    if (out_format == LDX_OUT_K16_RSQ || out_format == LDX_OUT_K16_DPRIME) {
        if (!fp4) {
            set_error("the one-measure cell formats run on the FP4 or the popcount kernel, not on the int8 matrix kernel");
            return LDX_E_UNSUPPORTED;
        }
        if (out_format == LDX_OUT_K16_RSQ)
            return launch_mfma<false, false, true, ldx_k16r>(alt, fa, fr, q, n_snps, n_hap, unit_begin, unit_end, (ldx_k16r *)out,
                                                            nullptr, nullptr, sched, s);
        return launch_mfma<false, false, true, ldx_k16d>(alt, fa, fr, q, n_snps, n_hap, unit_begin, unit_end, (ldx_k16d *)out,
                                                        nullptr, nullptr, sched, s);
    }
    if (out_format == LDX_OUT_R32) LDX_GO(false, false, ldx_r32);
    if (out_format == LDX_OUT_K16) {
        if (out_n11) LDX_GO(false, true, ldx_k16);
        LDX_GO(false, false, ldx_k16);
    }
    if (out_raw && out_n11) LDX_GO(true, true, ldx_ld32);
    if (out_raw) LDX_GO(true, false, ldx_ld32);
    if (out_n11) LDX_GO(false, true, ldx_ld32);
    LDX_GO(false, false, ldx_ld32);
#undef LDX_GO
}

int triangle_dosage_mfma(const void *alt, const double *gstat, uint32_t n_snps, uint32_t n_hap, uint64_t unit_begin,
                         uint64_t unit_end, ldx_r32 *out, void *workspace, hipStream_t s)
{
    return launch_mfma<false, false, true, ldx_r32, true>(alt, gstat, nullptr, nullptr, n_snps, n_hap, unit_begin, unit_end, out,
                                                          nullptr, nullptr, (uint32_t *)workspace, s);
}

}

namespace ldx {

__global__ void area_mask_kernel(const uint32_t *__restrict__ queries, uint32_t n_query, uint8_t *__restrict__ is_query)
{
    const uint32_t k = blockIdx.x * blockDim.x + threadIdx.x;
    if (k < n_query) is_query[queries[k]] = 1;
}

__global__ void __launch_bounds__(1024) area_band_plan_kernel(const int64_t *__restrict__ pos, uint32_t n_snps, uint32_t T,
                                                              int64_t flank, const uint32_t *__restrict__ queries,
                                                              uint32_t n_query, uint32_t *__restrict__ g_begin,
                                                              uint32_t *__restrict__ g_end, uint32_t *__restrict__ pass_base,
                                                              unsigned long long *__restrict__ n_hits, uint32_t *__restrict__ order,
                                                              uint32_t *__restrict__ first_base, uint32_t *__restrict__ sched)
{
    const uint32_t qmin = queries[0], qmax = queries[n_query - 1u];
    __shared__ unsigned long long carry;
    __shared__ unsigned long long wsum[16];
    constexpr uint32_t kCoarse = 4096;
    __shared__ int64_t tile_pos[kCoarse];
    const bool coarse = T <= kCoarse;
    if (coarse)
        for (uint32_t k = threadIdx.x; k < T; k += 1024u) tile_pos[k] = pos[k * kSlab];
    if (threadIdx.x == 0) { carry = 0; pass_base[0] = 0; first_base[0] = 0; store_agent(n_hits, 0ull); }
    if (threadIdx.x < 256u) store_agent(&sched[threadIdx.x], 0u);
    block_sync();
    for (uint32_t t0 = 0; t0 < T; t0 += 1024u) {
        const uint32_t t = t0 + threadIdx.x;
        uint32_t cnt = 0;
        if (t < T) {
            const uint32_t jlast = ((t + 1u) * kSlab < n_snps ? (t + 1u) * kSlab : n_snps) - 1u;
            const int64_t lim = pos[jlast] + flank;
            uint32_t lo = jlast + 1u, hi = n_snps;
            if (coarse) {
                uint32_t klo = t + 1u, khi = T;
                while (klo < khi) { const uint32_t m = (klo + khi) / 2; if (tile_pos[m] > lim) khi = m; else klo = m + 1u; }
                if (klo < T) hi = klo * kSlab;
                if (klo > t + 1u) lo = (klo - 1u) * kSlab + 1u;
            }
            while (lo < hi) { const uint32_t m = (lo + hi) / 2; if (pos[m] > lim) hi = m; else lo = m + 1u; }
            uint32_t ge = (lo + kRows64 - 1u) / kRows64;
            uint32_t gb = 2u * t;
            if (t * kSlab > qmax || jlast < qmin) {
                const uint32_t qb = qmin / kRows64, qe = qmax / kRows64 + 1u;
                gb = gb > qb ? gb : qb;
                ge = ge < qe ? ge : qe;
            }
            if (ge < gb) ge = gb;
            g_begin[t] = gb;
            g_end[t] = ge;
            cnt = (ge - gb + kMfmaWaves - 1u) / kMfmaWaves;
        }
        unsigned long long x = (unsigned long long)cnt | ((unsigned long long)(cnt != 0u) << 32);
        const uint32_t lane = threadIdx.x & 63u, wv = threadIdx.x >> 6;
#pragma unroll
        for (int off = 1; off < 64; off <<= 1) { const unsigned long long y = __shfl_up(x, off); if (lane >= (uint32_t)off) x += y; }
        if (lane == 63) wsum[wv] = x;
        block_sync();
        unsigned long long pre = 0;
        for (uint32_t k = 0; k < wv; ++k) pre += wsum[k];
        const unsigned long long incl = carry + pre + x;
        if (t < T) {
            pass_base[t + 1u] = (uint32_t)incl;
            first_base[t + 1u] = (uint32_t)(incl >> 32);
        }
        block_sync();
        if (threadIdx.x == 1023) carry = incl;
        block_sync();
    }
    if (!order) return;
    __threadfence_block();
    block_sync();
    for (uint32_t t = threadIdx.x; t < T; t += 1024u) {
        uint32_t a = 0, b = T;
        for (uint32_t xr = 0; xr < 8u; ++xr) {
            const uint32_t lo = (uint32_t)((uint64_t)T * xr / 8u), hi = (uint32_t)((uint64_t)T * (xr + 1u) / 8u);
            if (t >= lo && t < hi) { a = lo; b = hi; }
        }
        const uint32_t pb = pass_base[t], cnt = pass_base[t + 1u] - pb;
// ... 649 lines not shown
    LDX_REQUIRE(alt && acnt && rcnt && fa && fr && positions && sums && workspace, "null pointer");
    LDX_REQUIRE(n_annot <= 8u, "at most 8 annotation categories");
    LDX_REQUIRE(annot || n_annot == 0u, "annot is null but n_annot > 0");
    LDX_REQUIRE(n_snps >= 1 && n_hap >= 1 && window >= 0, "bad shape");
    if (const int rc = band_args_ok(__func__, workspace, workspace_bytes, ldx::score_mfma_workspace_bytes(n_snps),
                                    "ldx_ld_score_workspace_bytes", n_hap, path, "LD scores run", &window))
        return rc;
    return ldx::score_mfma(alt, acnt, rcnt, fa, fr, n_snps, n_hap, positions, window, annot, n_annot, path != LDX_PATH_MFMA, sums,
                           workspace, (hipStream_t)stream);
}

extern "C" int ldx_ld_cross_dev(const void *alt, const uint32_t *acnt, const uint32_t *rcnt, const double *fa, const double *fr,
                                uint32_t n_snps, uint32_t n_hap, const int64_t *positions, int64_t window, int path,
                                uint64_t *sides, uint64_t *cross, void *workspace, size_t workspace_bytes, void *stream)
{
    LDX_REQUIRE(alt && acnt && rcnt && fa && fr && positions && sides && cross && workspace, "null pointer");
    LDX_REQUIRE(n_snps >= 1 && n_hap >= 1 && window >= 0, "bad shape");
    if (const int rc = band_args_ok(__func__, workspace, workspace_bytes, ldx::score_mfma_workspace_bytes(n_snps),
                                    "ldx_ld_cross_workspace_bytes", n_hap, path, "the cross-LD profile runs", &window))
        return rc;
    const int rc = ldx::score_mfma(alt, acnt, rcnt, fa, fr, n_snps, n_hap, positions, window, nullptr, 0u, path != LDX_PATH_MFMA,
                                   sides, workspace, (hipStream_t)stream, true, __func__);
    if (rc != LDX_OK) return rc;
    return ldx_ld_cross_scan_dev(sides, n_snps, cross, stream);
}

namespace ldx {
typedef int v4i_p __attribute__((ext_vector_type(4)));
typedef int v16i_p __attribute__((ext_vector_type(16)));
template <int kVariant>
__global__ void __launch_bounds__(256) probe_mfma_kernel(uint32_t *__restrict__ sink, uint32_t iters)
{
    const uint32_t tid = blockIdx.x * blockDim.x + threadIdx.x;
    v4i_p a = {(int)(tid & 0x01010101u), 0x01000100, 0x00010001, 0x01010000};
    v4i_p b = {0x01010101, (int)((tid >> 3) & 0x01010101u), 0x00000101, 0x01000001};
    uint32_t s = 0;
    if (kVariant == 0) {
        v16i_p acc[8];
#pragma unroll
        for (int k = 0; k < 8; ++k)
#pragma unroll
            for (int e = 0; e < 16; ++e) acc[k][e] = 0;
        for (uint32_t it = 0; it < iters; ++it) {
#pragma unroll
            for (int k = 0; k < 8; ++k) acc[k] = __builtin_amdgcn_mfma_i32_32x32x32_i8(a, b, acc[k], 0, 0, 0);
        }
#pragma unroll
        for (int k = 0; k < 8; ++k)
#pragma unroll
            for (int e = 0; e < 16; ++e) s += (uint32_t)acc[k][e];
    } else {
        v4i_p acc[8];
#pragma unroll
        for (int k = 0; k < 8; ++k) acc[k] = v4i_p{0, 0, 0, 0};
        for (uint32_t it = 0; it < iters; ++it) {
#pragma unroll
            for (int k = 0; k < 8; ++k) acc[k] = __builtin_amdgcn_mfma_i32_16x16x64_i8(a, b, acc[k], 0, 0, 0);
        }
#pragma unroll
        for (int k = 0; k < 8; ++k) s += (uint32_t)(acc[k].x + acc[k].y + acc[k].z + acc[k].w);
    }
    sink[tid] = s;
}
}

extern "C" int ldx_probe_mfma_dev(uint32_t *sink, uint32_t blocks, uint32_t threads, uint32_t iters, int variant,
                                  void *stream)
{
    LDX_REQUIRE(sink && blocks >= 1 && threads >= 64 && threads <= 256 && threads % 64 == 0, "bad argument");
    if (variant == 0)
        ldx::probe_mfma_kernel<0><<<blocks, threads, 0, (hipStream_t)stream>>>(sink, iters);
    else
        ldx::probe_mfma_kernel<1><<<blocks, threads, 0, (hipStream_t)stream>>>(sink, iters);
    LDX_HIP(hipGetLastError());
    return LDX_OK;
}

extern "C" int ldx_debug_force_short_passes(int n_short)
{
    ldx::g_forced_short.store(n_short < 0 ? -1 : n_short, std::memory_order_relaxed);
    return LDX_OK;
}

extern "C" int ldx_debug_counters(uint64_t out[8], int reset)
{
    LDX_REQUIRE(out, "null pointer");
    LDX_HIP(hipDeviceSynchronize());
    LDX_HIP(hipMemcpyFromSymbol(out, HIP_SYMBOL(ldx::g_dbg), 8 * sizeof(uint64_t)));
    if (reset) {
        const uint64_t zero[8] = {0, 0, 0, 0, 0, 0, 0, 0};
        LDX_HIP(hipMemcpyToSymbol(HIP_SYMBOL(ldx::g_dbg), zero, sizeof(zero)));
    }
    return LDX_OK;
}
```

### ld_tools_amd/csrc/ldx_pairs.hip

```cpp
#include <atomic>

#include "ldx_common.h"
#include "ldx_tile.h"

namespace ldx {

__device__ inline uint32_t find_tile(uint64_t u, uint64_t G, uint32_t T)
{
    uint32_t lo = 0, hi = T;
    while (hi - lo > 1) {
        const uint32_t mid = (lo + hi) / 2;
        if (tile_base(mid, G) <= u) lo = mid; else hi = mid;
    }
    return lo;
}

template <bool kRaw, bool kN11, typename Cell>
__global__ void __launch_bounds__(kThreads)
triangle_kernel(const uint4 *__restrict__ alt, const double *__restrict__ fa, const double *__restrict__ fr,
                const double *__restrict__ q, uint32_t n_snps, uint32_t n_slabs, uint32_t nchunks, double n,
                double rn, uint64_t u_begin, uint64_t u_end, Cell *__restrict__ out, ldx_ld64 *__restrict__ raw,
                uint32_t *__restrict__ n11)
{
    extern __shared__ uint4 lds[];
// ... 390 lines not shown

extern "C" int ldx_get_triangle_path(void) { return g_triangle_path.load(std::memory_order_relaxed); }

static size_t tile_lds_bytes(uint32_t nchunks) { return (size_t)nchunks * kSlab * 16u; }

static int ensure_lds(const void *kernel, size_t bytes)
{
    LDX_HIP(hipFuncSetAttribute(kernel, hipFuncAttributeMaxDynamicSharedMemorySize, (int)bytes));
    return LDX_OK;
}

static int num_cus() { return device_cus(); }

template <bool kRaw, bool kN11, typename Cell>
static int launch_triangle(const void *alt, const double *fa, const double *fr, const double *q, uint32_t n_snps,
                           uint32_t n_hap, uint64_t unit_begin, uint64_t unit_end, Cell *out, ldx_ld64 *out_raw,
                           uint32_t *out_n11, hipStream_t s)
{
    const uint32_t nch = ldx::n_chunks(n_hap);
    const size_t lds = tile_lds_bytes(nch);
    int rc = ensure_lds((const void *)triangle_kernel<kRaw, kN11, Cell>, lds);
    if (rc) return rc;
    const uint64_t total = unit_end - unit_begin;
    uint64_t grid = (uint64_t)num_cus();
    const uint64_t max_grid = (total + kWaves - 1) / kWaves;
    if (grid > max_grid) grid = max_grid;
    triangle_kernel<kRaw, kN11, Cell><<<(uint32_t)grid, kThreads, lds, s>>>(
        (const uint4 *)alt, fa, fr, q, n_snps, ldx::n_slabs(n_snps), nch, (double)n_hap, 1.0 / (double)n_hap, unit_begin,
        unit_end, out, out_raw, out_n11);
    LDX_HIP(hipGetLastError());
    return LDX_OK;
}

extern "C" size_t ldx_triangle_workspace_bytes(void) { return ldx::triangle_mfma_workspace_bytes(); }

extern "C" int ldx_triangle_workspace_init_dev(void *workspace, size_t workspace_bytes, void *stream)
{
    LDX_REQUIRE(workspace, "null pointer");
    LDX_REQUIRE(workspace_bytes >= ldx::triangle_mfma_workspace_bytes(), "workspace too small (see ldx_triangle_workspace_bytes)");
    LDX_HIP(hipMemsetAsync(workspace, 0, ldx::triangle_mfma_workspace_bytes(), (hipStream_t)stream));
    return LDX_OK;
}

extern "C" int ldx_triangle_dev(const void *alt, const double *fa, const double *fr, const double *q,
                                uint32_t n_snps, uint32_t n_hap, uint64_t unit_begin, uint64_t unit_end,
                                ldx_ld32 *out, ldx_ld64 *out_raw, uint32_t *out_n11, void *stream)
{
    return ldx_triangle_ex_dev(alt, fa, fr, q, n_snps, n_hap, unit_begin, unit_end,
                               g_triangle_path.load(std::memory_order_relaxed), LDX_OUT_LD32, out, out_raw, out_n11, nullptr, 0,
                               stream);
}

extern "C" int ldx_triangle_ex_dev(const void *alt, const double *fa, const double *fr, const double *q,
                                   uint32_t n_snps, uint32_t n_hap, uint64_t unit_begin, uint64_t unit_end, int path,
                                   int out_format, void *out, ldx_ld64 *out_raw, uint32_t *out_n11, void *workspace,
                                   size_t workspace_bytes, void *stream)
{
    LDX_REQUIRE(!workspace || workspace_bytes >= ldx::triangle_mfma_workspace_bytes(),
                "workspace too small (see ldx_triangle_workspace_bytes)");
    LDX_REQUIRE(!workspace || ((uintptr_t)workspace & 255u) == 0, "workspace must be 256-byte aligned");
    LDX_REQUIRE(alt && fa && fr && q && out, "null pointer");
    LDX_REQUIRE(known_path(path), "unknown path");
    const bool one_measure = out_format == LDX_OUT_K16_RSQ || out_format == LDX_OUT_K16_DPRIME;
    LDX_REQUIRE(out_format == LDX_OUT_LD32 || out_format == LDX_OUT_K16 || one_measure || out_format == LDX_OUT_R32,
                "unknown output format");
    LDX_REQUIRE(out_format == LDX_OUT_LD32 || !out_raw, "out_raw needs LDX_OUT_LD32");
    LDX_REQUIRE(!one_measure || !out_n11, "the one-measure formats take no side output");
    LDX_REQUIRE(out_format != LDX_OUT_R32 || !out_n11, "LDX_OUT_R32 takes no side output");
    LDX_REQUIRE(n_snps >= 1 && n_hap >= 1, "bad shape");
    if (n_hap > LDX_MAX_HAPS) {
        set_error("ldx_triangle_dev: n_hap %u > LDX_MAX_HAPS %u", n_hap, LDX_MAX_HAPS);
        return LDX_E_UNSUPPORTED;
    }
    if (!check_recip(n_hap)) {
        set_error("ldx_triangle_dev: reciprocal division check failed for n = %u", n_hap);
        return LDX_E_UNSUPPORTED;
    }
    const uint64_t U = ldx_triangle_units(n_snps);
    if (unit_end > U) unit_end = U;
    if (unit_begin >= unit_end) return LDX_OK;
    hipStream_t s = (hipStream_t)stream;
    if (path != LDX_PATH_POPCOUNT) {
        const int rc = triangle_mfma(alt, fa, fr, q, n_snps, n_hap, unit_begin, unit_end, out_format, out, out_raw, out_n11,
                                     path != LDX_PATH_MFMA, workspace, s);
        if (rc != ldx::kNoMatrixPath) return rc;
        if (path != LDX_PATH_AUTO) return LDX_E_UNSUPPORTED;
    }
    if (out_format == LDX_OUT_R32)
        return launch_triangle<false, false>(alt, fa, fr, q, n_snps, n_hap, unit_begin, unit_end, (ldx_r32 *)out, out_raw, out_n11, s);
    if (out_format == LDX_OUT_K16_RSQ)
        return launch_triangle<false, false>(alt, fa, fr, q, n_snps, n_hap, unit_begin, unit_end, (ldx_k16r *)out, out_raw, out_n11, s);
    if (out_format == LDX_OUT_K16_DPRIME)
        return launch_triangle<false, false>(alt, fa, fr, q, n_snps, n_hap, unit_begin, unit_end, (ldx_k16d *)out, out_raw, out_n11, s);
    if (out_format == LDX_OUT_K16) {
        ldx_k16 *o = (ldx_k16 *)out;
        if (out_n11)
            return launch_triangle<false, true>(alt, fa, fr, q, n_snps, n_hap, unit_begin, unit_end, o, out_raw, out_n11, s);
        return launch_triangle<false, false>(alt, fa, fr, q, n_snps, n_hap, unit_begin, unit_end, o, out_raw, out_n11, s);
    }
    ldx_ld32 *o = (ldx_ld32 *)out;
    if (out_raw && out_n11)
        return launch_triangle<true, true>(alt, fa, fr, q, n_snps, n_hap, unit_begin, unit_end, o, out_raw, out_n11, s);
    if (out_raw)
        return launch_triangle<true, false>(alt, fa, fr, q, n_snps, n_hap, unit_begin, unit_end, o, out_raw, out_n11, s);
    if (out_n11)
        return launch_triangle<false, true>(alt, fa, fr, q, n_snps, n_hap, unit_begin, unit_end, o, out_raw, out_n11, s);
    return launch_triangle<false, false>(alt, fa, fr, q, n_snps, n_hap, unit_begin, unit_end, o, out_raw, out_n11, s);
}

extern "C" int ldx_pair_counts_dev(const void *alt_i, uint32_t n_i, const void *alt_j, uint32_t n_j,
                                   uint32_t n_hap, uint32_t *n11, size_t ld, void *stream)
{
    LDX_REQUIRE(alt_i && alt_j && n11, "null pointer");
    LDX_REQUIRE(n_i >= 1 && n_j >= 1 && n_hap >= 1 && ld >= n_j, "bad shape");
    if (n_hap > LDX_MAX_HAPS) {
        set_error("ldx_pair_counts_dev: n_hap %u > LDX_MAX_HAPS %u", n_hap, LDX_MAX_HAPS);
        return LDX_E_UNSUPPORTED;
    }
    const uint32_t nch = ldx::n_chunks(n_hap);
    const size_t lds = tile_lds_bytes(nch);
    int rc = ensure_lds((const void *)pair_counts_kernel, lds);
    if (rc) return rc;
    const uint32_t tiles_j = ldx::n_slabs(n_j);
    const uint32_t groups_i = (n_i + kGroup - 1) / kGroup;
    uint32_t gy = (groups_i + kWaves - 1) / kWaves;
    const uint32_t want = (uint32_t)(num_cus() + tiles_j - 1) / tiles_j;
    if (gy > want) gy = want;
    if (gy < 1) gy = 1;
    pair_counts_kernel<<<dim3(tiles_j, gy), kThreads, lds, (hipStream_t)stream>>>(
        (const uint4 *)alt_i, (const uint4 *)alt_j, n_i, n_j, nch, n11, ld);
    LDX_HIP(hipGetLastError());
    return LDX_OK;
}

extern "C" int ldx_ld_from_counts_ex_dev(uint32_t n, size_t m, const uint32_t *n11, const uint32_t *a1,
                                         const uint32_t *r1, const uint32_t *a2, const uint32_t *r2, ldx_ld64 *raw,
                                         double *k, ldx_ld32 *cells32, ldx_k16 *cells16, uint8_t *flags, void *stream)
{
    LDX_REQUIRE(n11 && a1 && r1 && a2 && r2, "null pointer");
    LDX_REQUIRE(n >= 1, "n must be positive (the reference raises ZeroDivisionError, calc_ld.py:33)");
    if (m == 0) return LDX_OK;
    if (!check_recip(n)) {
        set_error("ldx_ld_from_counts_dev: reciprocal division check failed for n = %u", n);
        return LDX_E_UNSUPPORTED;
    }
    ld_from_counts_kernel<<<(uint32_t)((m + 255) / 256), 256, 0, (hipStream_t)stream>>>(
        (double)n, 1.0 / (double)n, m, n11, a1, r1, a2, r2, raw, k, cells32, cells16, flags);
    LDX_HIP(hipGetLastError());
    return LDX_OK;
}

extern "C" int ldx_ld_from_counts_dev(uint32_t n, size_t m, const uint32_t *n11, const uint32_t *a1,
                                      const uint32_t *r1, const uint32_t *a2, const uint32_t *r2,
                                      ldx_ld64 *raw, ldx_ld32 *rounded, uint8_t *flags, void *stream)
{
    return ldx_ld_from_counts_ex_dev(n, m, n11, a1, r1, a2, r2, raw, nullptr, rounded, nullptr, flags, stream);
}

extern "C" int ldx_ld_pairs_dev(const void *alt, const uint32_t *acnt, const uint32_t *rcnt, uint32_t n_snps,
                                uint32_t n_hap, const uint32_t *rows, const uint32_t *cols, size_t m, double *k,
                                ldx_ld64 *raw, uint8_t *flags, uint32_t *n11, void *stream)
{
    LDX_REQUIRE(alt && acnt && rcnt && rows && cols, "null pointer");
    LDX_REQUIRE(n_snps >= 1 && n_hap >= 1, "bad shape");
    if (m == 0) return LDX_OK;
    ld_pairs_kernel<<<(uint32_t)((m + 3) / 4), 256, 0, (hipStream_t)stream>>>(
        (const uint4 *)alt, acnt, rcnt, n_snps, ldx::n_chunks(n_hap), (double)n_hap, rows, cols, m, k, raw, flags, n11);
// ... 85 lines not shown
```

### ld_tools_amd/ops.py

```python
from __future__ import annotations

import ctypes
from dataclasses import dataclass
from typing import Optional, Sequence, Tuple

import numpy as np
import torch

from . import _lib
from ._lib import MEASURES, UNIT_PAIRS, check, lib
from .panel import PackedPanel, _ptr, _stream_ptr, require_gpu


PATHS = {"auto": 0, "popcount": 1, "mfma": 2, "fp4": 3}


def set_triangle_path(name: str) -> None:
    check(lib.ldx_set_triangle_path(PATHS[name]), "ldx_set_triangle_path")


def get_triangle_path() -> str:
    code = lib.ldx_get_triangle_path()
    return next(k for k, v in PATHS.items() if v == code)

# ... 122 lines not shown
                raise _lib.LdxError("escape cells need the panel (TriangleResult.panel) to be resolved")
            ex = ld_pairs(self.panel, rr + r0, cc)
            col = 0 if measure == "r_square" else 1
            for a, b, k in zip((rr + r0).tolist(), cc.tolist(), ex["k"][:, col].tolist()):
                v = k / 10000.0
                fixes[(a, b)] = 0 if (thres is not None and v < thres) else v
        return d, fixes

    @property
    def unsharded(self) -> bool:
        return self.unit_begin == 0 and self.unit_end == lib.ldx_triangle_units(self.n_snps)

    def _rounded_only(self, what: str) -> None:
        if self.r32 is not None:
            raise _lib.LdxError(f"{what}() reads a rounded measure; an r32 result holds signed r (use r_matrix())")

    def r_matrix(self, rows: Optional[Tuple[int, int]] = None, cols: Optional[Tuple[int, int]] = None) -> torch.Tensor:
        if self.r32 is None:
            raise _lib.LdxError(f"r_matrix() needs an r32 result (this one is {self.fmt})")
        if not self.unsharded:
            raise _lib.LdxError("r_matrix() needs an unsharded TriangleResult")
        if self.panel is None:
            raise _lib.LdxError("r_matrix() needs the panel (TriangleResult.panel) for the diagonal")
        n = self.n_snps
        r0, r1 = rows if rows is not None else (0, n)
        c0, c1 = cols if cols is not None else (0, n)
        if not (0 <= r0 <= r1 <= n and 0 <= c0 <= c1 <= n):
            raise _lib.LdxError(f"r_matrix(): block {rows} x {cols} outside the {n} x {n} matrix")
        out = torch.empty((r1 - r0, c1 - c0), dtype=torch.float32, device=self.r32.device)
        if out.numel():
            p = self.panel
            if self.dosage:
                check(lib.ldx_triangle_r_block_dosage_dev(self.r32.data_ptr(), n, p.dosage_stats()[1].data_ptr(), r0, r1, c0, c1,
                                                          out.data_ptr(), c1 - c0, _stream_ptr()),
                      "ldx_triangle_r_block_dosage_dev")
                return out
            check(lib.ldx_triangle_r_block_dev(self.r32.data_ptr(), n, p.acnt.data_ptr(), p.rcnt.data_ptr(), p.n_hap,
                                               r0, r1, c0, c1, out.data_ptr(), c1 - c0, _stream_ptr()),
                  "ldx_triangle_r_block_dev")
        return out


def ld_triangle(panel: PackedPanel, unit_range: Optional[Tuple[int, int]] = None, want_raw: bool = False,
                want_n11: bool = False, out: Optional[TriangleResult] = None, fmt: str = "ld32",
                path: Optional[str] = None, dosage: bool = False) -> TriangleResult:
    total = panel.n_units
    u0, u1 = (0, total) if unit_range is None else unit_range
    u0, u1 = max(0, u0), min(total, u1)
    cells = max(0, u1 - u0) * UNIT_PAIRS
    dev = panel.device
    if fmt not in _lib.FORMATS:
        raise _lib.LdxError(f"unknown cell format {fmt!r}")
    if fmt != "ld32" and want_raw:
        raise _lib.LdxError("the unrounded output travels with the ld32 format only")
    if fmt in _lib.ONE_MEASURE and want_n11:
        raise _lib.LdxError("the one-measure formats take no side output")
    if fmt == "r32" and want_n11:
        raise _lib.LdxError("the r32 format takes no side output")
    if dosage:
        if fmt != "r32":
            raise _lib.LdxError(f"ld_triangle: dosage=True needs fmt='r32' (got {fmt!r}): the rounded measures are haplotype statistics")
        if unit_range is not None:
            raise _lib.LdxError("ld_triangle: dosage=True does not take unit_range (no sharded dosage triangle)")
        if panel.n_hap % 2:
            raise _lib.LdxError(f"ld_triangle: dosage=True needs an even n_hap (got {panel.n_hap}): individual k owns haplotypes 2k and 2k + 1")
    if out is not None and out.dosage != bool(dosage):
        raise _lib.LdxError("ld_triangle: `out` was made with another `dosage`")
    if out is None:
        out = TriangleResult(panel.n_snps, u0, u1,
                             torch.empty((cells, 2), dtype=torch.float32, device=dev) if fmt == "ld32" else None,
                             torch.empty((cells, 2), dtype=torch.float64, device=dev) if want_raw else None,
                             torch.empty(cells, dtype=torch.int32, device=dev) if want_n11 else None,
                             torch.empty((cells, 2), dtype=torch.int16, device=dev) if fmt == "k16" else None,
                             k16one=torch.empty(cells, dtype=torch.int16, device=dev) if fmt in _lib.ONE_MEASURE else None,
                             one_fmt=fmt if fmt in _lib.ONE_MEASURE else None,
                             r32=torch.empty(cells, dtype=torch.float32, device=dev) if fmt == "r32" else None,
                             dosage=bool(dosage))
    elif (out.n_snps, out.unit_begin, out.unit_end, out.fmt) != (panel.n_snps, u0, u1, fmt):
        raise _lib.LdxError("ld_triangle: `out` has a different shape or format")
    out.panel = panel
    if cells:
        pcode = lib.ldx_get_triangle_path() if path is None else PATHS[path]
        if out.ws is None and pcode != PATHS["popcount"]:
            out.ws = torch.zeros(lib.ldx_triangle_workspace_bytes(), dtype=torch.uint8, device=dev)
        if dosage:
            check(lib.ldx_triangle_dosage_dev(panel.alt.data_ptr(), panel.dosage_stats()[1].data_ptr(), panel.n_snps, panel.n_hap,
                                              u0, u1, pcode, out.r32.data_ptr(), _ptr(out.ws),
                                              0 if out.ws is None else out.ws.numel(), _stream_ptr()), "ldx_triangle_dosage_dev")
            return out
        check(lib.ldx_triangle_ex_dev(panel.alt.data_ptr(), panel.fa.data_ptr(), panel.fr.data_ptr(),
                                      panel.q.data_ptr(), panel.n_snps, panel.n_hap, u0, u1, pcode,
                                      _lib.FORMATS[fmt], out.cells.data_ptr(), _ptr(out.raw), _ptr(out.n11),
                                      _ptr(out.ws), 0 if out.ws is None else out.ws.numel(), _stream_ptr()),
              "ldx_triangle_ex_dev")
    return out


def pair_counts(panel_i: PackedPanel, panel_j: Optional[PackedPanel] = None) -> torch.Tensor:
    pj = panel_j or panel_i
    if pj.n_hap != panel_i.n_hap:
        raise _lib.LdxError("pair_counts: panels differ in haplotype count")
    out = torch.empty((panel_i.n_snps, pj.n_snps), dtype=torch.int32, device=panel_i.device)
    check(lib.ldx_pair_counts_dev(panel_i.alt.data_ptr(), panel_i.n_snps, pj.alt.data_ptr(), pj.n_snps,
                                  panel_i.n_hap, out.data_ptr(), pj.n_snps, _stream_ptr()),
          "ldx_pair_counts_dev")
    return out


def ld_pairs(panel: PackedPanel, rows, cols) -> dict:
    dev = panel.device
    r = torch.as_tensor(np.ascontiguousarray(np.asarray(rows, dtype=np.int64).astype(np.int32))).to(dev)
    c = torch.as_tensor(np.ascontiguousarray(np.asarray(cols, dtype=np.int64).astype(np.int32))).to(dev)
    m = int(r.numel())
    if int(c.numel()) != m:
        raise _lib.LdxError("ld_pairs: rows and cols differ in length")
    k = torch.empty((m, 2), dtype=torch.float64, device=dev)
    raw = torch.empty((m, 2), dtype=torch.float64, device=dev)
    flags = torch.empty(m, dtype=torch.uint8, device=dev)
    n11 = torch.empty(m, dtype=torch.int32, device=dev)
    if m:
        check(lib.ldx_ld_pairs_dev(panel.alt.data_ptr(), panel.acnt.data_ptr(), panel.rcnt.data_ptr(), panel.n_snps,
                                   panel.n_hap, r.data_ptr(), c.data_ptr(), m, k.data_ptr(), raw.data_ptr(),
                                   flags.data_ptr(), n11.data_ptr(), _stream_ptr()), "ldx_ld_pairs_dev")
    return {"k": k.cpu().numpy(), "raw": raw.cpu().numpy(), "flags": flags.cpu().numpy(),
            "n11": n11.cpu().numpy().view(np.uint32)}


def ld_from_counts(n: int, n11, a1, r1, a2, r2, device: Optional[torch.device] = None, full: bool = False):
    dev = device or torch.device("cuda", torch.cuda.current_device())
    def up(x):
        t = torch.as_tensor(np.ascontiguousarray(np.asarray(x, dtype=np.uint32)).view(np.int32))
        return t.to(dev)
    t11, ta1, tr1, ta2, tr2 = (up(x) for x in (n11, a1, r1, a2, r2))
    m = t11.numel()
    raw = torch.empty((m, 2), dtype=torch.float64, device=dev)
    rnd = torch.empty((m, 2), dtype=torch.float32, device=dev)
    flags = torch.empty(m, dtype=torch.uint8, device=dev)
    k = torch.empty((m, 2), dtype=torch.float64, device=dev) if full else None
    k16 = torch.empty((m, 2), dtype=torch.int16, device=dev) if full else None
    check(lib.ldx_ld_from_counts_ex_dev(int(n), m, t11.data_ptr(), ta1.data_ptr(), tr1.data_ptr(), ta2.data_ptr(),
                                        tr2.data_ptr(), raw.data_ptr(), _ptr(k), rnd.data_ptr(), _ptr(k16),
                                        flags.data_ptr(), _stream_ptr()), "ldx_ld_from_counts_ex_dev")
    sure32 = (flags & 0x80) != 0
    flags = flags & 3
    if full:
        return raw, rnd, flags, k, k16, sure32
    return raw, rnd, flags


class AreaHits:

    def __init__(self, query: torch.Tensor, oppos: torch.Tensor, ld32: torch.Tensor, n_pairs, offsets=None,
                 band_passes=None):
        self.query = query
        self.oppos = oppos
        self.ld32 = ld32
        self._n_pairs = n_pairs
        self.offsets = offsets
        self._band_passes = band_passes

    @property
    def n_pairs(self) -> int:
        if callable(self._n_pairs):
            self._n_pairs = self._n_pairs()
        return self._n_pairs

    @property
# ... 3028 lines not shown
```

Baseline: 448.7 billion.

## Split tail passes along K into slices with a reduction epilogue

```diff
diff --git a/include/ldx.h b/include/ldx.h
--- a/include/ldx.h
+++ b/include/ldx.h
@@ -110,6 +110,7 @@
 int ldx_set_triangle_path(int path);
 int ldx_get_triangle_path(void);
 size_t ldx_triangle_workspace_bytes(void);
+size_t ldx_triangle_workspace_bytes_ex(uint32_t n_snps, uint32_t n_hap, uint64_t unit_begin, uint64_t unit_end);
 int ldx_triangle_workspace_init_dev(void *workspace, size_t workspace_bytes, void *stream);
 int ldx_triangle_ex_dev(const void *alt, const double *fa, const double *fr, const double *q,
                         uint32_t n_snps, uint32_t n_hap, uint64_t unit_begin, uint64_t unit_end,
@@ -370,6 +371,7 @@
                        void *stream);
 
 int ldx_debug_force_short_passes(int n_short);
+int ldx_debug_force_k_split(int n_split, int n_slices);
 int ldx_debug_counters(uint64_t out[8], int reset);
 
 #ifdef __cplusplus
diff --git a/ld_tools_amd/_lib.py b/ld_tools_amd/_lib.py
--- a/ld_tools_amd/_lib.py
+++ b/ld_tools_amd/_lib.py
@@ -101,6 +101,8 @@
     "ldx_triangle_dev": (_int, [_vp, _vp, _vp, _vp, _u32, _u32, _u64, _u64, _vp, _vp, _vp, _vp]),
     "ldx_triangle_ex_dev": (_int, [_vp, _vp, _vp, _vp, _u32, _u32, _u64, _u64, _int, _int, _vp, _vp, _vp, _vp, _sz, _vp]),
     "ldx_triangle_workspace_bytes": (_sz, []),
+    "ldx_triangle_workspace_bytes_ex": (_sz, [_u32, _u32, _u64, _u64]),
+    "ldx_debug_force_k_split": (_int, [_int, _int]),
     "ldx_triangle_workspace_init_dev": (_int, [_vp, _sz, _vp]),
     "ldx_triangle_dense_ex_dev": (_int, [_vp, _int, _u32, _int, _int, _dbl, _u32, _u32, _vp, _sz, _vp]),
     "ldx_triangle_r_block_dev": (_int, [_vp, _u32, _vp, _vp, _u32, _u32, _u32, _u32, _u32, _vp, _sz, _vp]),
diff --git a/ld_tools_amd/build.py b/ld_tools_amd/build.py
--- a/ld_tools_amd/build.py
+++ b/ld_tools_amd/build.py
@@ -13,7 +13,7 @@
            "ldx_select.hip", "ldx_band.hip", "ldx_rect.hip", "ldx_em.hip", "ldx_pwc.hip", "ldx_pwband.hip",
            "ldx_emband.hip", "ldx_bed.hip", "ldx_gabriel.hip", "ldx_king.hip", "ldx_geno.hip"]
 HEADERS = [CSRC / "ldx_common.h", CSRC / "ldx_fp4.h", CSRC / "ldx_tile.h", CSRC / "ldx_pwc_tile.h", CSRC / "ldx_em_tile.h",
-           CSRC / "ldx_em_pw_tile.h", CSRC / "ldx_band_plan.h", CSRC / "ldx_sample_store.h",
+           CSRC / "ldx_em_pw_tile.h", CSRC / "ldx_band_plan.h", CSRC / "ldx_sample_store.h", CSRC / "ldx_tail_plan.h",
            PKG.parent / "include" / "ldx.h"]
 
 FLAGS = ["-O3", "-std=c++17", "-fPIC", "-shared", "--offload-arch=gfx950", "-ffp-contract=off",
diff --git a/ld_tools_amd/csrc/ldx_common.h b/ld_tools_amd/csrc/ldx_common.h
--- a/ld_tools_amd/csrc/ldx_common.h
+++ b/ld_tools_amd/csrc/ldx_common.h
@@ -33,9 +33,10 @@
 constexpr int kNoMatrixPath = -1000;
 
 size_t triangle_mfma_workspace_bytes();
+size_t triangle_mfma_workspace_bytes_ex(uint32_t n_snps, uint32_t n_hap, uint64_t unit_begin, uint64_t unit_end);
 int triangle_mfma(const void *alt, const double *fa, const double *fr, const double *q, uint32_t n_snps, uint32_t n_hap,
                   uint64_t unit_begin, uint64_t unit_end, int out_format, void *out, ldx_ld64 *out_raw, uint32_t *out_n11,
-                  bool fp4, void *workspace, hipStream_t s);
+                  bool fp4, void *workspace, size_t workspace_bytes, hipStream_t s);
 
 size_t area_mfma_workspace_bytes(uint32_t n_snps);
 int area_mfma(const void *alt, const double *fa, const double *fr, const double *q, uint32_t n_snps, uint32_t n_hap,
diff --git a/ld_tools_amd/csrc/ldx_mfma.hip b/ld_tools_amd/csrc/ldx_mfma.hip
--- a/ld_tools_amd/csrc/ldx_mfma.hip
+++ b/ld_tools_amd/csrc/ldx_mfma.hip
@@ -7,6 +7,7 @@
 #include "ldx_common.h"
 #include "ldx_fp4.h"
 #include "ldx_tile.h"
+#include "ldx_tail_plan.h"
 
 namespace ldx {
 
@@ -30,6 +31,17 @@
 {
     const void *t;
     asm volatile("s_mov_b64 %1, %3\n\tglobal_load_dwordx2 %0, %2, %1" : "=v"(dst), "=&s"(t) : "v"(voff), "s"(sbase));
+}
+
+__device__ __forceinline__ void gstore16_agent_s(void *sbase, uint32_t voff, v4u v)
+{
+    void *t;
+    asm volatile("s_mov_b64 %0, %3\n\tglobal_store_dwordx4 %1, %2, %0 sc1" : "=&s"(t) : "v"(voff), "v"(v), "s"(sbase) : "memory");
+}
+__device__ __forceinline__ void gload16_agent_s(v4u &dst, uint32_t voff, const void *sbase)
+{
+    const void *t;
+    asm volatile("s_mov_b64 %1, %3\n\tglobal_load_dwordx4 %0, %2, %1 sc1" : "=v"(dst), "=&s"(t) : "v"(voff), "s"(sbase) : "memory");
 }
 
 #ifndef LDX_STEP_UNROLL
@@ -116,6 +128,10 @@
 constexpr uint32_t kCuSlots = 2048;
 constexpr uint32_t kSchedWords = 3u + kCuSlots;
 constexpr size_t kTriWorkspaceBytes = (kSchedWords * 4u + 255u) / 256u * 256u;
+constexpr uint32_t kReadyWord = 128, kArrivedWord = 256;
+static_assert(kTailHeadBytes == kTriWorkspaceBytes && kArrivedWord + kTailMaxSplit <= kSchedWords && kTailMaxSplit <= 8u * 32u,
+              "the split passes' counters live in the workspace's head");
+static std::atomic<int> g_forced_split{-1}, g_forced_slices{0};
 __device__ unsigned long long g_dbg[8];
 #if defined(LDX_TUNING) && !defined(LDX_STAMPS_ONLY)
 #define LDX_COUNT(slot, v) do { if (lane == 0) atomicAdd(&g_dbg[slot], (unsigned long long)(v)); } while (0)
@@ -304,7 +320,12 @@
     static_assert((kSweep != 0) == (kScore || kProd), "kSweep: the words (Score, Cross) or right-hand sides (Prod) per accumulator sweep");
     static_assert(!kCross || kSweep == 1, "the one-sided sums are the score band's column 0, rows and columns apart");
     const uint32_t p_end = kArea ? aa.pass_base[n_slabs] : p_end_arg;
-    const uint32_t n_norm = p_end - p_begin - n_short, n_tickets = n_norm + 2u * n_short;
+    constexpr bool kSplit = kFp4 && !kRaw && !kN11 && kOp == BandOp::None && !std::is_same<Cell, ldx_r32>::value;
+    const uint32_t n_split = kSplit ? (uint32_t)aa.hit_cap & 0xFFFFu : 0u, n_slices = kSplit ? (uint32_t)(aa.hit_cap >> 16) & 0xFFFFu : 1u;
+    const uint32_t split0 = p_end - p_begin - n_split;
+    const uint32_t n_norm = p_end - p_begin - n_short - n_split, n_tickets = n_norm + 2u * n_short + n_split * n_slices;
+    unsigned char *const part_base = reinterpret_cast<unsigned char *>(aa.hits);
+    constexpr uint32_t kEpiTicket = 0x80000000u;
 #if defined(LDX_TUNING) && !defined(LDX_STAMPS_ONLY)
     int ablate = ablate_arg;
     if (ablate_arg & 64) ablate = (blockIdx.x < (gridDim.x + 1) / 2) ? 5 : 2;
@@ -379,6 +400,20 @@
     const F32Const fc32 = aa.f32;
     const uint32_t my_xcd = kArea ? (__builtin_amdgcn_s_getreg(63508) & 7u) : 0u;
     uint32_t static_next = blockIdx.x;
+    auto draw_epi = [&]() -> uint32_t {
+        unsigned long long *const ready = reinterpret_cast<unsigned long long *>(sched + kReadyWord);
+        const uint32_t nw = (n_split + 31u) / 32u;
+        for (uint32_t w = 0; w < nw; ++w) {
+            unsigned long long v = __hip_atomic_load(&ready[w], __ATOMIC_RELAXED, __HIP_MEMORY_SCOPE_AGENT);
+            while (v) {
+                const uint32_t b = (uint32_t)__builtin_ctzll(v);
+                const unsigned long long old = atomicAnd(&ready[w], ~(1ull << b));
+                if ((old >> b) & 1ull) return kEpiTicket | (w * 64u + b);
+                v = old & ~(1ull << b);
+            }
+        }
+        return 0xFFFFFFFFu;
+    };
     auto draw = [&]() -> uint32_t {
         if constexpr (kArea) {
             for (uint32_t k = 0; k < 8u; ++k) {
@@ -391,7 +426,11 @@
             return 0xFFFFFFFFu;
         } else {
             if (!sched) return static_next += gridDim.x;
-            return gridDim.x + atomicAdd(&sched[0], 1u);
+            const uint32_t got = gridDim.x + atomicAdd(&sched[0], 1u);
+            if constexpr (kSplit) {
+                if (n_split && got >= n_tickets) return draw_epi();
+            }
+            return got;
         }
     };
     uint32_t *ktok = nullptr;
@@ -410,7 +449,8 @@
         block_sync();
         const uint32_t ticket = tickets[parity];
         parity ^= 1u;
-        if (kArea ? ticket == 0xFFFFFFFFu : ticket >= n_tickets) {
+        const bool epi_ticket = kSplit && ticket >= kEpiTicket && ticket != 0xFFFFFFFFu;
+        if (kArea ? ticket == 0xFFFFFFFFu : (ticket >= n_tickets && !epi_ticket)) {
             if (tid == 0 && sched && atomicAdd(&sched[1], 1u) == gridDim.x - 1u) {
                 store_agent(&sched[1], 0u);
                 if (kArea)
@@ -420,9 +460,17 @@
             }
             break;
         }
-        const bool short_pass = !kArea && ticket >= n_norm;
-        const uint32_t hsel = short_pass ? (ticket - n_norm) & 1u : 0u;
-        const uint32_t seq = short_pass ? n_norm + ((ticket - n_norm) >> 1) : ticket;
+        const bool slice_ticket = kSplit && !epi_ticket && ticket >= n_norm + 2u * n_short;
+        const uint32_t slice_r = slice_ticket ? ticket - (n_norm + 2u * n_short) : 0u;
+        const uint32_t split_p = epi_ticket ? (ticket & ~kEpiTicket) >> 1 : (slice_ticket ? slice_r / n_slices : 0u);
+        const uint32_t slice_s = slice_ticket ? slice_r - split_p * n_slices : 0u;
+        const bool short_pass = !kArea && !slice_ticket && (epi_ticket || ticket >= n_norm);
+        const uint32_t hsel = epi_ticket ? ticket & 1u : (short_pass ? (ticket - n_norm) & 1u : 0u);
+        uint32_t seq = short_pass ? n_norm + ((ticket - n_norm) >> 1) : ticket;
+        if constexpr (kSplit) {
+            if (slice_ticket || epi_ticket) seq = split0 + split_p;
+            else if (seq >= split0) seq += n_split;
+        }
         uint32_t p = p_begin + seq;
         auto pbase = [&](uint32_t tile) { return kArea ? aa.pass_base[tile] : mfma_pass_base(tile, n_slabs); };
         auto tile_of_pass = [&](uint32_t pp) {
@@ -451,7 +499,7 @@
             t = tile_of_pass(p);
         }
         const bool new_tile = t != t_prev;
-        t_prev = t;
+        t_prev = slice_ticket ? 0xFFFFFFFFu : t;
         const uint64_t tb = base64(t), te = base64(t + 1u);
         const uint64_t area_first = kArea ? tb + (aa.g_begin[t] - 2u * t) : 0u;
         const uint64_t pass = (kArea ? area_first : tb) + (uint64_t)(p - pbase(t)) * kMfmaWaves;
@@ -460,8 +508,15 @@
         const uint32_t b_off = kFp4 ? ((tid >> 7) * kSlab + (tid & 127u)) * 16u : (tid >> 1) * kBRow + (tid & 1u) * 64u;
         const uint32_t nblocks = kFp4 ? nchunks / 2u : nchunks;
 
-        auto pass_body = [&](auto mm_c) {
+        auto pass_body = [&](auto mm_c, auto kind_c) {
             constexpr int MM = decltype(mm_c)::value;
+            constexpr bool kSlice = decltype(kind_c)::value == 1, kEpi = decltype(kind_c)::value == 2;
+            static_assert(!kSlice || (kSplit && MM == 2), "K-slices: the fp32-tier triangle, whole height");
+            static_assert(!kEpi || (kSplit && MM == 1), "epilogue tickets: the fp32-tier triangle, half height");
+            [[maybe_unused]] const uint32_t split_pu = (kSlice || kEpi) ? __builtin_amdgcn_readfirstlane(split_p) : 0u;
+            const uint32_t slice_su = kSlice ? __builtin_amdgcn_readfirstlane(slice_s) : 0u;
+            [[maybe_unused]] const uint32_t kb0 = kSlice ? tail_slice_begin(slice_su, n_slices, nblocks) : 0u;
+            [[maybe_unused]] const uint32_t nb_slice = kSlice ? tail_slice_begin(slice_su + 1u, n_slices, nblocks) - kb0 : 0u;
             const uint64_t vv = pass + wave;
             const bool active = vv >= seg_begin && vv < seg_end;
             const uint32_t g64 = (uint32_t)((vv < te ? vv : pass) - tb) + 2u * t;
@@ -538,12 +593,18 @@
             };
             typedef std::conditional_t<kFp4, v4u, v2u> bring_t;
             bring_t br[3];
-            auto clampc = [&](uint32_t c) { return c < nblocks ? c : nblocks - 1u; };
+            auto clampc = [&](uint32_t c) {
+                if constexpr (kSlice) return c < nb_slice ? c : nb_slice - 1u;
+                else return c < nblocks ? c : nblocks - 1u;
+            };
             constexpr uint32_t kBlockBytes = kAStride * 16u;
             const uint32_t b_voff = kFp4 ? (uint32_t)((((size_t)t * nchunks + (tid >> 7)) * kSlab + (tid & 127u)) * 16u)
                                          : (uint32_t)(((size_t)t * nchunks * kSlab) * 16u + tid * 8u);
             const uint32_t a_voff = (uint32_t)((size_t)(ai - alt) * 16u);
-            auto block_base = [&](uint32_t blk) { return reinterpret_cast<const unsigned char *>(alt) + (size_t)blk * kBlockBytes; };
+            auto block_base = [&](uint32_t blk) {
+                if constexpr (kSlice) return reinterpret_cast<const unsigned char *>(alt) + (size_t)(blk + kb0) * kBlockBytes;
+                else return reinterpret_cast<const unsigned char *>(alt) + (size_t)blk * kBlockBytes;
+            };
             auto load_b = [&](bring_t &dst, uint32_t blk) {
                 if constexpr (kFp4) gload16_s(dst, b_voff, block_base(blk));
                 else gload8_s(dst, b_voff, block_base(blk));
@@ -564,7 +625,7 @@
                 if constexpr (kFp4) return expand32_a4(x);
                 else return EXPAND_A(x);
             };
-            {
+            if constexpr (!kEpi) {
                 bring_t w0;
                 load_b(w0, 0u);
                 load_b(br[1], clampc(1));
@@ -633,7 +694,7 @@
                 const uint32_t i = row0 + (MM == 1 ? l32 : lane);
                 const R32Snp r = snp_ars(i);
                 if (lane < kStatRows) *reinterpret_cast<d2s *>(rstat + lane * kStat) = d2s{r.a, r.rs};
-            } else if (!kRaw) {
+            } else if (!kRaw && !kSlice) {
                 if (new_tile && tid < kSlab) {
                     const uint32_t j = t * kSlab + tid;
                     const FastCol c = fast_col(fa[j], fr[j], n);
@@ -692,7 +753,7 @@
 #pragma unroll
             for (int m = 0; m < MM; ++m) af0[m] = expand_a(ar[0][m].x);
 
-            const uint32_t nch_run = (ablate & 2) ? 1u : nblocks;
+            const uint32_t nch_run = kSlice ? nb_slice : kEpi ? 0u : (ablate & 2) ? 1u : nblocks;
 #ifdef LDX_CHUNK_STAMPS
             unsigned long long cst[6] = {0, 0, 0, 0, 0, 0};
 #endif
@@ -804,6 +865,42 @@
 #endif
             LDX_STAMP(2);
             uint32_t next_ticket = 0;
+            if constexpr (kSlice) {
+                if (counting) {
+                    uint32_t ln = lane;
+                    asm volatile("" : "+v"(ln));
+                    unsigned char *const pw = part_base + ((size_t)(split_pu * n_slices + slice_su) * kMfmaWaves + wave) * (kTailTileBytes / kMfmaWaves);
+#pragma unroll
+                    for (int k = 0; k < 4 * MM; ++k)
+#pragma unroll
+                        for (int qd = 0; qd < 4; ++qd) {
+                            const acc_t &a = acc[k >> 2][k & 3];
+                            const v4f v = {a[4 * qd], a[4 * qd + 1], a[4 * qd + 2], a[4 * qd + 3]};
+                            gstore16_agent_s(pw + (uint32_t)(k * 4 + qd) * 1024u, ln * 16u, __builtin_bit_cast(v4u, v));
+                        }
+                }
+                asm volatile("s_waitcnt vmcnt(0)" ::: "memory");
+                block_sync();
+                if (tid == 0) {
+                    if (ktok) atomicExch(ktok, 0u);
+                    if (atomicAdd(&sched[kArrivedWord + split_p], 1u) == n_slices - 1u) {
+                        store_agent(&sched[kArrivedWord + split_p], 0u);
+                        atomicOr(reinterpret_cast<unsigned long long *>(sched + kReadyWord) + (split_p >> 5), 3ull << (2u * (split_p & 31u)));
+                    }
+                    next_ticket = draw();
+                }
+                if (tid == 0) tickets[parity] = next_ticket;
+#ifdef LDX_TUNING
+                LDX_STAMP(3);
+                ++npass;
+                if (my_stamps && lane == 0) {
+                    my_stamps[3] = npass;
+                    my_stamps[4] = __builtin_amdgcn_s_memrealtime();
+                    my_stamps[5] = __builtin_amdgcn_s_memtime();
+                }
+#endif
+                return;
+            }
             if (tid == 0) {
                 if (ktok) atomicExch(ktok, 0u);
                 next_ticket = draw();
@@ -815,6 +912,50 @@
             } else if (!active) {
                 if (tid == 0) tickets[parity] = next_ticket;
                 return;
+            }
+            if constexpr (kEpi) {
+                if (counting) {
+                    uint32_t ln = lane;
+                    asm volatile("" : "+v"(ln));
+                    const unsigned char *const pw = part_base + ((size_t)(split_pu * n_slices) * kMfmaWaves + wave) * (kTailTileBytes / kMfmaWaves) +
+                                                    __builtin_amdgcn_readfirstlane(hsel) * 16u * 1024u;
+                    v4u pa[16], pb[16];
+                    auto load_part = [&](v4u (&d)[16], uint32_t s) {
+#pragma unroll
+                        for (int k = 0; k < 16; ++k) gload16_agent_s(d[k], ln * 16u, pw + (size_t)s * kTailTileBytes + (uint32_t)k * 1024u);
+                    };
+                    auto add_part = [&](v4u (&d)[16]) {
+#pragma unroll
+                        for (int k = 0; k < 16; ++k) {
+                            asm volatile("" : "+v"(d[k]));
+                            const v4f v = __builtin_bit_cast(v4f, d[k]);
+                            acc[0][k >> 2][4 * (k & 3)] += v.x;
+                            acc[0][k >> 2][4 * (k & 3) + 1] += v.y;
+                            acc[0][k >> 2][4 * (k & 3) + 2] += v.z;
+                            acc[0][k >> 2][4 * (k & 3) + 3] += v.w;
+                        }
+                    };
+                    asm volatile("s_waitcnt vmcnt(0)" ::: "memory");
+                    load_part(pa, 0u);
+                    for (uint32_t s = 0; s < n_slices; s += 2u) {
+                        if (s + 1u < n_slices) {
+                            load_part(pb, s + 1u);
+                            asm volatile("s_waitcnt vmcnt(16)" ::: "memory");
+                        } else {
+                            asm volatile("s_waitcnt vmcnt(0)" ::: "memory");
+                        }
+                        add_part(pa);
+                        if (s + 1u < n_slices) {
+                            if (s + 2u < n_slices) {
+                                load_part(pa, s + 2u);
+                                asm volatile("s_waitcnt vmcnt(16)" ::: "memory");
+                            } else {
+                                asm volatile("s_waitcnt vmcnt(0)" ::: "memory");
+                            }
+                            add_part(pb);
+                        }
+                    }
+                }
             }
             typedef double d2 __attribute__((ext_vector_type(2)));
             double fa2[4], fr2[4];
@@ -1759,13 +1900,23 @@
             finish_pass(std::true_type{});
         };
         if constexpr (kArea) {
-            pass_body(std::integral_constant<int, 2>{});
+            pass_body(std::integral_constant<int, 2>{}, std::integral_constant<int, 0>{});
         } else {
 #ifdef LDX_MM1
-            pass_body(std::integral_constant<int, 1>{});
+            pass_body(std::integral_constant<int, 1>{}, std::integral_constant<int, 0>{});
 #else
-            if (short_pass) pass_body(std::integral_constant<int, 1>{});
-            else pass_body(std::integral_constant<int, 2>{});
+            if constexpr (kSplit) {
+                if (slice_ticket) {
+                    pass_body(std::integral_constant<int, 2>{}, std::integral_constant<int, 1>{});
+                    continue;
+                }
+                if (epi_ticket) {
+                    pass_body(std::integral_constant<int, 1>{}, std::integral_constant<int, 2>{});
+                    continue;
+                }
+            }
+            if (short_pass) pass_body(std::integral_constant<int, 1>{}, std::integral_constant<int, 0>{});
+            else pass_body(std::integral_constant<int, 2>{}, std::integral_constant<int, 0>{});
 #endif
         }
     }
@@ -1791,25 +1942,14 @@
 #undef LDX_BAND_SWEEP_BEGIN
 #undef LDX_BAND_SWEEP_END
 
-template <bool kRaw, bool kN11, bool kFp4, typename Cell, bool kDosage = false>
-static int launch_mfma(const void *alt, const double *fa, const double *fr, const double *q, uint32_t n_snps,
-                       uint32_t n_hap, uint64_t unit_begin, uint64_t unit_end, Cell *out, ldx_ld64 *out_raw,
-                       uint32_t *out_n11, uint32_t *sched, hipStream_t s)
-{
-    const uint32_t nch = n_chunks(n_hap);
-    if (plane_check("ld_triangle on the matrix pipe", nullptr, n_snps, n_hap)) return kNoMatrixPath;
-    const size_t lds = mfma_lds_bytes(kStatRows, kFp4 && !kRaw && !kN11 && !std::is_same<Cell, ldx_r32>::value);
-    if (lds > 64u * 1024u) {
-        static std::atomic<uint64_t> opted{0};
-        int dev = 0;
-        LDX_HIP(hipGetDevice(&dev));
-        if (dev < 0 || dev >= 64 || !((opted.load(std::memory_order_relaxed) >> dev) & 1u)) {
-            LDX_HIP(hipFuncSetAttribute((const void *)triangle_mfma_kernel<kRaw, kN11, BandOp::None, kFp4, Cell, 0, kDosage>,
-                                        hipFuncAttributeMaxDynamicSharedMemorySize, (int)lds));
-            if (dev >= 0 && dev < 64) opted.fetch_or(1ull << dev, std::memory_order_relaxed);
-        }
-    }
-    const int cus = device_cus();
+struct TriTickets {
+    uint32_t p_begin, p_end;
+    uint64_t slots;
+    TailPlan unsplit, split;
+};
+static TriTickets tri_tickets(uint32_t n_snps, uint32_t n_hap, uint64_t unit_begin, uint64_t unit_end, bool fp4)
+{
+    TriTickets k{};
     const uint32_t ns = n_slabs(n_snps);
     const uint64_t G64 = (uint64_t)ns * 2u;
     auto base64 = [&](uint64_t t) { return t * G64 - t * (t - 1u); };
@@ -1823,21 +1963,73 @@
     };
     const uint64_t v_begin = unit_begin / 8u, v_end = (unit_end + 7u) / 8u;
     const uint32_t t0 = tile_of(v_begin), t1 = tile_of(v_end - 1u);
-    const uint32_t p_begin = mfma_pass_base(t0, ns) + (uint32_t)((v_begin - base64(t0)) / kMfmaWaves);
-    const uint32_t p_end = mfma_pass_base(t1, ns) + (uint32_t)((v_end - base64(t1) + kMfmaWaves - 1u) / kMfmaWaves);
-    const uint64_t slots = (uint64_t)cus * kWgPerCu;
-    const uint32_t n_pass = p_end - p_begin;
-    uint32_t n_short = 2ull * n_pass <= slots ? n_pass : (n_pass > slots ? (uint32_t)(slots / 4u) : 0u);
+    k.p_begin = mfma_pass_base(t0, ns) + (uint32_t)((v_begin - base64(t0)) / kMfmaWaves);
+    k.p_end = mfma_pass_base(t1, ns) + (uint32_t)((v_end - base64(t1) + kMfmaWaves - 1u) / kMfmaWaves);
+    k.slots = (uint64_t)device_cus() * kWgPerCu;
+    const uint32_t n_pass = k.p_end - k.p_begin;
+    k.unsplit = tail_plan_unsplit(n_pass, (uint32_t)k.slots);
     const int forced = g_forced_short.load(std::memory_order_relaxed);
-    if (forced >= 0) n_short = (uint32_t)forced < n_pass ? (uint32_t)forced : n_pass;
+    if (forced >= 0) k.unsplit.n_short = (uint32_t)forced < n_pass ? (uint32_t)forced : n_pass;
 #ifdef LDX_MM1
-    n_short = n_pass;
-#endif
-    uint64_t grid = slots;
-    if (grid > (uint64_t)n_pass + n_short) grid = (uint64_t)n_pass + n_short;
+    k.unsplit.n_short = n_pass;
+    return k;
+#endif
+    const uint32_t max_split = fp4 ? n_pass : 0u;
+    const uint32_t nblocks = n_chunks(n_hap) / 2u;
+    const int f_split = g_forced_split.load(std::memory_order_relaxed);
+    if (f_split >= 0) {
+        uint32_t S = (uint32_t)g_forced_slices.load(std::memory_order_relaxed);
+        if (S > kTailMaxSlices) S = kTailMaxSlices;
+        if (S > nblocks) S = nblocks;
+        uint32_t n = (uint32_t)f_split < n_pass ? (uint32_t)f_split : n_pass;
+        if (S >= 2u && n > kTailMaxTiles / S) n = kTailMaxTiles / S;
+        if (fp4 && S >= 2u && n) {
+            const uint32_t rest = n_pass - n;
+            k.split = TailPlan{n, S, k.unsplit.n_short < rest ? k.unsplit.n_short : rest};
+        }
+    } else if (fp4 && forced < 0) {
+        k.split = tail_plan(n_pass, (uint32_t)k.slots, nblocks, max_split);
+    }
+#ifdef LDX_TUNING
+    if (getenv("LDX_ABLATE") && (atoi(getenv("LDX_ABLATE")) & 4096)) k.split = TailPlan{};
+#endif
+    return k;
+}
+
+template <bool kRaw, bool kN11, bool kFp4, typename Cell, bool kDosage = false>
+static int launch_mfma(const void *alt, const double *fa, const double *fr, const double *q, uint32_t n_snps,
+                       uint32_t n_hap, uint64_t unit_begin, uint64_t unit_end, Cell *out, ldx_ld64 *out_raw,
+                       uint32_t *out_n11, uint32_t *sched, size_t workspace_bytes, hipStream_t s)
+{
+    const uint32_t nch = n_chunks(n_hap);
+    if (plane_check("ld_triangle on the matrix pipe", nullptr, n_snps, n_hap)) return kNoMatrixPath;
+    const size_t lds = mfma_lds_bytes(kStatRows, kFp4 && !kRaw && !kN11 && !std::is_same<Cell, ldx_r32>::value);
+    if (lds > 64u * 1024u) {
+        static std::atomic<uint64_t> opted{0};
+        int dev = 0;
+        LDX_HIP(hipGetDevice(&dev));
+        if (dev < 0 || dev >= 64 || !((opted.load(std::memory_order_relaxed) >> dev) & 1u)) {
+            LDX_HIP(hipFuncSetAttribute((const void *)triangle_mfma_kernel<kRaw, kN11, BandOp::None, kFp4, Cell, 0, kDosage>,
+                                        hipFuncAttributeMaxDynamicSharedMemorySize, (int)lds));
+            if (dev >= 0 && dev < 64) opted.fetch_or(1ull << dev, std::memory_order_relaxed);
+        }
+    }
+    const TriTickets tk = tri_tickets(n_snps, n_hap, unit_begin, unit_end, kFp4);
+    const uint32_t p_begin = tk.p_begin, p_end = tk.p_end, n_pass = p_end - p_begin;
+    constexpr bool kSplit = kFp4 && !kRaw && !kN11 && !std::is_same<Cell, ldx_r32>::value;
+    const bool split = kSplit && sched && tk.split.n_split && workspace_bytes >= tail_workspace_bytes(tk.split);
+    const TailPlan plan = split ? tk.split : tk.unsplit;
+    const uint32_t n_short = plan.n_short;
+    uint64_t grid = tk.slots;
+    const uint64_t n_tickets = (uint64_t)(n_pass - plan.n_split - n_short) + 2ull * n_short + (uint64_t)plan.n_split * plan.S;
+    if (grid > n_tickets) grid = n_tickets;
     if (grid < 1) grid = 1;
     AreaArgs tri_args{};
     tri_args.f32 = f32_const((double)n_hap);
+    if (plan.n_split) {
+        tri_args.hits = reinterpret_cast<ldx_hit *>(reinterpret_cast<unsigned char *>(sched) + kTailHeadBytes);
+        tri_args.hit_cap = (uint64_t)plan.n_split | ((uint64_t)plan.S << 16);
+    }
     int ablate = 0;
     unsigned long long *stamps = nullptr;
 #ifdef LDX_TUNING
@@ -1874,16 +2066,27 @@
 
 size_t triangle_mfma_workspace_bytes() { return kTriWorkspaceBytes; }
 
+size_t triangle_mfma_workspace_bytes_ex(uint32_t n_snps, uint32_t n_hap, uint64_t unit_begin, uint64_t unit_end)
+{
+    if (n_snps == 0 || n_hap == 0) return kTriWorkspaceBytes;
+    if ((uint64_t)n_slabs(n_snps) * kSlab * n_chunks(n_hap) * 16u >= (1ull << 32)) return kTriWorkspaceBytes;
+    const uint64_t U = ldx_triangle_units(n_snps);
+    if (unit_end > U) unit_end = U;
+    if (unit_begin >= unit_end) return kTriWorkspaceBytes;
+    const TriTickets tk = tri_tickets(n_snps, n_hap, unit_begin, unit_end, true);
+    return tk.split.n_split ? tail_workspace_bytes(tk.split) : kTriWorkspaceBytes;
+}
+
 int triangle_mfma(const void *alt, const double *fa, const double *fr, const double *q, uint32_t n_snps, uint32_t n_hap,
                   uint64_t unit_begin, uint64_t unit_end, int out_format, void *out, ldx_ld64 *out_raw, uint32_t *out_n11,
-                  bool fp4, void *workspace, hipStream_t s)
+                  bool fp4, void *workspace, size_t workspace_bytes, hipStream_t s)
 {
     uint32_t *const sched = (uint32_t *)workspace;
 #define LDX_GO(R, N, CELL)                                                                                          \
     return fp4 ? launch_mfma<R, N, true, CELL>(alt, fa, fr, q, n_snps, n_hap, unit_begin, unit_end, (CELL *)out,    \
-                                               out_raw, out_n11, sched, s)                                          \
+                                               out_raw, out_n11, sched, workspace_bytes, s)                                          \
                : launch_mfma<R, N, false, CELL>(alt, fa, fr, q, n_snps, n_hap, unit_begin, unit_end, (CELL *)out,   \
-                                                out_raw, out_n11, sched, s)
+                                                out_raw, out_n11, sched, workspace_bytes, s)
     if (out_format == LDX_OUT_K16_RSQ || out_format == LDX_OUT_K16_DPRIME) {
         if (!fp4) {
             set_error("the one-measure cell formats run on the FP4 or the popcount kernel, not on the int8 matrix kernel");
@@ -1891,9 +2094,9 @@
         }
         if (out_format == LDX_OUT_K16_RSQ)
             return launch_mfma<false, false, true, ldx_k16r>(alt, fa, fr, q, n_snps, n_hap, unit_begin, unit_end, (ldx_k16r *)out,
-                                                            nullptr, nullptr, sched, s);
+                                                            nullptr, nullptr, sched, workspace_bytes, s);
         return launch_mfma<false, false, true, ldx_k16d>(alt, fa, fr, q, n_snps, n_hap, unit_begin, unit_end, (ldx_k16d *)out,
-                                                        nullptr, nullptr, sched, s);
+                                                        nullptr, nullptr, sched, workspace_bytes, s);
     }
     if (out_format == LDX_OUT_R32) LDX_GO(false, false, ldx_r32);
     if (out_format == LDX_OUT_K16) {
@@ -1911,7 +2114,7 @@
                          uint64_t unit_end, ldx_r32 *out, void *workspace, hipStream_t s)
 {
     return launch_mfma<false, false, true, ldx_r32, true>(alt, gstat, nullptr, nullptr, n_snps, n_hap, unit_begin, unit_end, out,
-                                                          nullptr, nullptr, (uint32_t *)workspace, s);
+                                                          nullptr, nullptr, (uint32_t *)workspace, workspace ? kTriWorkspaceBytes : 0u, s);
 }
 
 }
@@ -2727,6 +2930,18 @@
     return LDX_OK;
 }
 
+extern "C" int ldx_debug_force_k_split(int n_split, int n_slices)
+{
+    ldx::g_forced_slices.store(n_slices < 0 ? 0 : n_slices, std::memory_order_relaxed);
+    ldx::g_forced_split.store(n_split < 0 ? -1 : n_split, std::memory_order_relaxed);
+    return LDX_OK;
+}
+
+extern "C" size_t ldx_triangle_workspace_bytes_ex(uint32_t n_snps, uint32_t n_hap, uint64_t unit_begin, uint64_t unit_end)
+{
+    return ldx::triangle_mfma_workspace_bytes_ex(n_snps, n_hap, unit_begin, unit_end);
+}
+
 extern "C" int ldx_debug_counters(uint64_t out[8], int reset)
 {
     LDX_REQUIRE(out, "null pointer");
diff --git a/ld_tools_amd/csrc/ldx_pairs.hip b/ld_tools_amd/csrc/ldx_pairs.hip
--- a/ld_tools_amd/csrc/ldx_pairs.hip
+++ b/ld_tools_amd/csrc/ldx_pairs.hip
@@ -496,7 +496,7 @@
     hipStream_t s = (hipStream_t)stream;
     if (path != LDX_PATH_POPCOUNT) {
         const int rc = triangle_mfma(alt, fa, fr, q, n_snps, n_hap, unit_begin, unit_end, out_format, out, out_raw, out_n11,
-                                     path != LDX_PATH_MFMA, workspace, s);
+                                     path != LDX_PATH_MFMA, workspace, workspace ? workspace_bytes : 0u, s);
         if (rc != ldx::kNoMatrixPath) return rc;
         if (path != LDX_PATH_AUTO) return LDX_E_UNSUPPORTED;
     }
diff --git a/ld_tools_amd/csrc/ldx_tail_plan.h b/ld_tools_amd/csrc/ldx_tail_plan.h
--- /dev/null
+++ b/ld_tools_amd/csrc/ldx_tail_plan.h
@@ -0,0 +1,128 @@
+#pragma once
+
+#include <stddef.h>
+#include <stdint.h>
+
+namespace ldx {
+
+constexpr double kTailWhole = 1.0, kTailHalf = 0.55, kTailEpi = 0.22;
+constexpr double tail_slice_cost(uint32_t S) { return 0.6 / (double)S + 0.03; }
+
+constexpr uint32_t kTailMaxSlices = 8;
+constexpr uint32_t kTailMaxSplit = 256;
+constexpr uint32_t kTailMaxTiles = 256;
+constexpr size_t kTailHeadBytes = 8448;
+constexpr size_t kTailTileBytes = 4u * 32768u;
+
+struct TailPlan {
+    uint32_t n_split;
+    uint32_t S;
+    uint32_t n_short;
+};
+
+constexpr size_t tail_workspace_bytes(const TailPlan &p)
+{
+    return kTailHeadBytes + (size_t)p.n_split * p.S * kTailTileBytes;
+}
+
+constexpr uint32_t tail_slice_begin(uint32_t s, uint32_t S, uint32_t nblocks) { return s * nblocks / S; }
+
+inline TailPlan tail_plan_unsplit(uint32_t n_pass, uint32_t slots)
+{
+    const uint32_t n_short = 2ull * n_pass <= slots ? n_pass : (n_pass > slots ? slots / 4u : 0u);
+    return TailPlan{0u, 0u, n_short < n_pass ? n_short : n_pass};
+}
+
+struct TailSim {
+    static constexpr int kMaxGroups = 64;
+    double t[kMaxGroups];
+    uint32_t c[kMaxGroups];
+    int ng = 0;
+    double last_end = 0.0;
+
+    void add(double time, uint32_t count)
+    {
+        for (int g = 0; g < ng; ++g)
+            if (t[g] == time) { c[g] += count; return; }
+        if (ng == kMaxGroups) {
+            int l = 0;
+            for (int g = 1; g < ng; ++g) if (t[g] > t[l]) l = g;
+            if (time > t[l]) t[l] = time;
+            c[l] += count;
+            return;
+        }
+        t[ng] = time;
+        c[ng++] = count;
+    }
+    void run(uint64_t n, double cost)
+    {
+        while (n) {
+            int f = 0;
+            for (int g = 1; g < ng; ++g) if (t[g] < t[f]) f = g;
+            const uint32_t k = n < c[f] ? (uint32_t)n : c[f];
+            const double t0 = t[f];
+            c[f] -= k;
+            if (c[f] == 0) { t[f] = t[ng - 1]; c[f] = c[ng - 1]; --ng; }
+            last_end = t0 + cost;
+            add(last_end, k);
+            n -= k;
+        }
+    }
+    double end() const
+    {
+        double e = 0.0;
+        for (int g = 0; g < ng; ++g) if (c[g] && t[g] > e) e = t[g];
+        return e;
+    }
+};
+
+inline double tail_makespan(const TailPlan &p, uint32_t n_pass, uint32_t slots)
+{
+    if (slots == 0 || n_pass == 0) return 0.0;
+    TailSim sim;
+    const uint64_t n_whole = (uint64_t)n_pass - p.n_split - p.n_short;
+    const uint64_t q = n_whole / slots, r = n_whole % slots;
+    if (r) sim.add((double)(q + 1u) * kTailWhole, (uint32_t)r);
+    sim.add((double)q * kTailWhole, slots - (uint32_t)r);
+    sim.run(2ull * p.n_short, kTailHalf);
+    if (p.n_split) {
+        sim.run((uint64_t)p.n_split * p.S, tail_slice_cost(p.S));
+        const double slices_end = sim.last_end;
+        sim.run(2ull * p.n_split, kTailEpi);
+        const double e = sim.end();
+        return e > slices_end + kTailEpi ? e : slices_end + kTailEpi;
+    }
+    return sim.end();
+}
+
+inline TailPlan tail_plan(uint32_t n_pass, uint32_t slots, uint32_t nblocks, uint32_t max_split)
+{
+    TailPlan best = tail_plan_unsplit(n_pass, slots);
+    if (n_pass == 0 || slots == 0) return best;
+    double best_end = tail_makespan(best, n_pass, slots);
+    if (max_split > n_pass) max_split = n_pass;
+    if (max_split > kTailMaxSplit) max_split = kTailMaxSplit;
+    const uint32_t s_max = nblocks < kTailMaxSlices ? nblocks : kTailMaxSlices;
+    if (s_max < 2u || max_split == 0u) return best;
+    const uint32_t s_cand[4] = {2u, 4u, 8u, s_max};
+    for (uint32_t S : s_cand) {
+        if (S > s_max) continue;
+        const uint32_t cap = kTailMaxTiles / S < max_split ? kTailMaxTiles / S : max_split;
+        const uint32_t n_cand[6] = {slots / 32u, slots / 16u, slots / 8u, slots / 4u, slots / 2u, cap};
+        for (uint32_t ns : n_cand) {
+            if (ns > cap) ns = cap;
+            if (ns == 0u) continue;
+            const uint32_t rest = n_pass - ns;
+            const uint32_t h_cand[4] = {0u, slots / 8u, slots / 4u, 2ull * n_pass <= slots ? rest : 0u};
+            for (uint32_t nh : h_cand) {
+                if (nh > rest) nh = rest;
+                const TailPlan p{ns, S, nh};
+                const double e = tail_makespan(p, n_pass, slots);
+                if (e < best_end - 1e-9) { best_end = e; best = p; }
+            }
+        }
+    }
+    return best;
+}
+
+}
diff --git a/ld_tools_amd/ops.py b/ld_tools_amd/ops.py
--- a/ld_tools_amd/ops.py
+++ b/ld_tools_amd/ops.py
@@ -228,7 +228,10 @@
     if cells:
         pcode = lib.ldx_get_triangle_path() if path is None else PATHS[path]
         if out.ws is None and pcode != PATHS["popcount"]:
-            out.ws = torch.zeros(lib.ldx_triangle_workspace_bytes(), dtype=torch.uint8, device=dev)
+            head = lib.ldx_triangle_workspace_bytes()
+            need = head if dosage or pcode == PATHS["mfma"] else lib.ldx_triangle_workspace_bytes_ex(panel.n_snps, panel.n_hap, u0, u1)
+            out.ws = torch.empty(max(head, need), dtype=torch.uint8, device=dev)
+            out.ws[:head].zero_()
         if dosage:
             check(lib.ldx_triangle_dosage_dev(panel.alt.data_ptr(), panel.dosage_stats()[1].data_ptr(), panel.n_snps, panel.n_hap,
                                               u0, u1, pcode, out.r32.data_ptr(), _ptr(out.ws),
```

New measurement: 119.0 billion. -73.5%, worse.
